# Gabriel-SGama/Semantic-SuperPoint

Hardware: AMD Instinct MI355X
Metric: image-pairs/sec at 240x320 bs32 (pair training step) (higher is better)
Workload: dtype f32

## Files before the change

include/ssp_hip.h:

```cpp
#ifndef SSP_HIP_H
#define SSP_HIP_H

#include <stddef.h>
#include <stdint.h>

#ifdef __cplusplus
extern "C" {
#endif

typedef struct ssp_handle ssp_handle;

enum { SSP_ARCH_GAUSS2 = 0, SSP_ARCH_GAUSS2_SSMALL = 1 };
enum { SSP_NREP = 32 };

typedef struct {
  int arch;
  int n_classes;
  int max_batch;
  int height;
  int width;
  int n_match;
  int n_non;
  int dense_loss;
} ssp_config;
// ... 231 lines not shown
                      int cap, int n_pairs, int pair_stride, float nn_thresh, void* workspace_dev, float* match_dev,
                      int32_t* n_match_dev, void* stream);

#define SSP_CLASS_NONE 255
int ssp_op_point_classes(const float* sout_nhwc_dev, int cs, int b, int h, int w, int n_classes, const float* pts_dev,
                         int pts_stride, const int32_t* count_dev, int cap, uint8_t* cls_dev, void* stream);
int ssp_point_classes(ssp_handle* h, int slot, int n, const float* pts_dev, int pts_stride, const int32_t* count_dev, int cap,
                      uint8_t* cls_dev, void* stream);
size_t ssp_filter_workspace_bytes(int n, int cap);
int ssp_op_filter_points(const float* pts_dev, const int32_t* count_dev, const float* desc_dev, const uint8_t* cls_dev,
                         const uint32_t keep_mask[8], int n, int cap, float* pts_out_dev, int32_t* count_out_dev,
                         float* desc_out_dev, uint8_t* cls_out_dev, void* workspace_dev, void* stream);
int ssp_match_two_way_classes(const float* desc1_dev, const int32_t* count1_dev, const float* desc2_dev,
                              const int32_t* count2_dev, const uint8_t* cls1_dev, const uint8_t* cls2_dev, int cap, int n_pairs,
                              int pair_stride, float nn_thresh, void* workspace_dev, float* match_dev, int32_t* n_match_dev,
                              void* stream);

int ssp_eval_repeatability(const double* pts1_dev, const int32_t* n1_dev, const double* pts2_dev, const int32_t* n2_dev,
                           int cap, int n_pairs, int pair_stride, const double* hom_dev, const double* hom_inv_dev,
                           int height, int width, int keep_k, double dist_thresh, double* out_dev, void* stream);
size_t ssp_eval_ransac_workspace_bytes(int cap, int n_pairs);
int ssp_eval_ransac(const double* pts1_dev, const double* pts2_dev, int cap, int n_pairs, int pair_stride,
                    const float* match_dev, const int32_t* n_match_dev, const uint64_t* seeds_dev, void* workspace_dev,
                    double* h_dev, uint8_t* mask_dev, int32_t* n_inlier_dev, int32_t* status_dev, double* ap_dev,
                    void* stream);

#define SSP_DET_EVAL_MAX_R2 64
#define SSP_DET_EVAL_STATE_WORDS 80
#define SSP_DET_EVAL_CURVE_TILE 1024
typedef struct ssp_det_eval_params {
  int32_t height, width;
  float remove_zero;
  int32_t r2;
  float prob_thresh;
  int32_t simplified;
} ssp_det_eval_params;
size_t ssp_det_eval_workspace_bytes(const ssp_det_eval_params* p, int b, int cap);
int ssp_op_det_tp_fp(const float* prob_dev, const void* labels_dev, int labels_u8, const ssp_det_eval_params* p, int b,
                     void* workspace_dev, int64_t* keys_dev, int64_t capacity, int64_t* state_dev, void* stream);
int ssp_op_det_tp_fp_points(const float* pts_dev, const int32_t* count_dev, int cap, const void* labels_dev, int labels_u8,
                            const ssp_det_eval_params* p, int b, void* workspace_dev, int64_t* keys_dev, int64_t capacity,
                            int64_t* state_dev, void* stream);
size_t ssp_det_pr_curve_workspace_bytes(int64_t n_records);
int ssp_op_det_pr_curve(const int64_t* sorted_keys_dev, int64_t n_records, const int64_t* state_dev, void* workspace_dev,
                        float* prob_dev, uint8_t* tp_dev, double* precision_dev, double* recall_dev, double* map_dev,
                        void* stream);

#define SSP_TRACK_MAX_LENGTH 16
size_t ssp_track_workspace_bytes(int max_length, int point_cap, int row_cap);
int ssp_op_track_update(const int32_t* ids_in_dev, const int32_t* tid_in_dev, const double* score_in_dev,
                        const int32_t* state_in_dev, const float* match_dev, const double* match_score64_dev,
                        const int32_t* n_match_dev, const int32_t* n_points_dev, int max_length, int point_cap, int row_cap,
                        void* workspace_dev, int32_t* ids_out_dev, int32_t* tid_out_dev, double* score_out_dev,
                        int32_t* state_out_dev, void* stream);
int ssp_op_track_select(const int32_t* ids_dev, const int32_t* tid_dev, const double* score_dev, const int32_t* state_dev,
                        int max_length, int row_cap, int min_length, void* workspace_dev, double* tracks_dev,
                        int32_t* n_tracks_dev, void* stream);
int ssp_op_track_points(const double* tracks_dev, const int32_t* n_tracks_dev, const double* pts_dev, const int32_t* state_dev,
                        int max_length, int point_cap, int track_cap, int first_slot, double* xy_dev, void* stream);

int ssp_op_bn_bwd(const float* y_dev, const float* dout_dev, const float* gamma_dev, const float* stats4_dev,
                  float* dy_dev, float* dgamma_dev, float* dbeta_dev, float* dbias_dev, double* sums_dev, int n, int h,
                  int w, int c, int relu, int pool, void* stream);
int ssp_op_bn_bwd_strided(const float* y_dev, const float* dout_dev, const float* gamma_dev, const float* stats4_dev,
                          float* dy_dev, float* dgamma_dev, float* dbeta_dev, float* dbias_dev, double* sums_dev, int n,
                          int h, int w, int c, int cs, int relu, int pool, void* stream);

int ssp_set_conv_algo(int algo);
int ssp_handle_set_conv_algo(ssp_handle* h, int algo);

int ssp_debug_conv_knobs(int ablate, int grid);
int ssp_debug_occupancy(int which);

int ssp_debug_buffer(ssp_handle* h, int slot, const char* name, float** ptr, size_t* nfloats);

int ssp_debug_backward_taps(ssp_handle* h, float* arena_dev, size_t arena_floats, unsigned layer_mask);
size_t ssp_debug_backward_tap_floats(const ssp_handle* h, unsigned layer_mask);
int ssp_debug_backward_tap(ssp_handle* h, int slot, int layer, int which, size_t* offset, size_t* nfloats, unsigned* route);

int ssp_op_sparse_loss(const float* desc_a_nhwc_dev, const float* desc_b_nhwc_dev, const int32_t* match_a_dev,
                       const int32_t* match_b_dev, const int32_t* nonmatch_b_dev, int b, int hc, int wc, int n_match,
                       int n_non, int method, int dist, float coef_pos, float coef_neg, float* dd_a_nhwc_dev, float* dd_b_nhwc_dev,
                       float* out2_dev, void* stream);

int ssp_op_dense_loss(const float* desc_a_nhwc_dev, const float* desc_b_nhwc_dev, const float* homographies_dev,
                      const float* valid_dev, int b, int hc, int wc, float lamda_d, float descriptor_dist, int multi_task,
                      float scale, void* scratch_dev, size_t scratch_bytes, float* out3_dev, float* dda_dev,
                      float* ddb_dev, void* stream);

#ifdef __cplusplus
}
#endif
#endif
```

semantic-superpoint_amd/csrc/bn_kernels.hip.h:

```cpp
#pragma once
#include <hip/hip_runtime.h>
#include <stdint.h>

#include "conv_mfma.hip.h"

namespace sspk {

template <typename T>
__device__ __forceinline__ float4 ld4(const T* p) {
  if constexpr (sizeof(T) == 4) {
    return *reinterpret_cast<const float4*>(p);
  } else {
    const u32x2 v = *reinterpret_cast<const u32x2*>(p);
    return make_float4(bf16_lo(v[0]), bf16_hi(v[0]), bf16_lo(v[1]), bf16_hi(v[1]));
  }
}
template <typename T>
__device__ __forceinline__ void st4(T* p, float4 v) {
  if constexpr (sizeof(T) == 4) {
    *reinterpret_cast<float4*>(p) = v;
  } else {
    u32x2 o;
    o[0] = pack_bf16(v.x, v.y);
    o[1] = pack_bf16(v.z, v.w);
// ... 684 lines not shown
      for (int o = 16; o > 0; o >>= 1) part += __shfl_xor(part, o);
      s2 = part;
    }
    if (!writer) continue;
    const float k1 = (float)(s1 / a.count), k2 = (float)(s2 / a.count);
    float* k12 = const_cast<float*>(a.k12);
    k12[c] = k1;
    k12[C + c] = k2;
    if (dbeta != nullptr) dbeta[c] += (float)s1;
    if (dgamma != nullptr) dgamma[c] += (float)s2;
    if (a.dbias != nullptr) a.dbias[c] += a.gamma[c] * a.invstd[c] * (float)(s1 - a.count * (double)k1);
  }
}
template <typename T = float>
__global__ void bn_bwd_sums_kernel(const BnBwdArgs a0, const BnBwdArgs a1, int nviews, float* __restrict__ dgamma,
                                   float* __restrict__ dbeta) {
  bn_bwd_sums_body<T>(a0, a1, nviews, dgamma, dbeta);
}
struct BnSumsJobs {
  BnBwdArgs a0[3], a1[3];
  float* dgamma[3];
  float* dbeta[3];
  int n;
};
template <typename T = float>
__global__ void bn_bwd_sums_multi_kernel(const BnSumsJobs J, int nviews) {
  const int j = blockIdx.y;
  bn_bwd_sums_body<T>(J.a0[j], J.a1[j], nviews, J.dgamma[j], J.dbeta[j]);
}

__global__ void nhwc_affine_to_nchw_kernel(const float* __restrict__ y, const float* __restrict__ scale,
                                           const float* __restrict__ shift, float* __restrict__ out, int N, int HW,
                                           int C, int cs, int co) {
  const long idx = (long)blockIdx.x * blockDim.x + threadIdx.x;
  if (idx >= (long)N * C * HW) return;
  const int p = (int)(idx % HW);
  const int c = (int)((idx / HW) % C);
  const int n = (int)(idx / ((long)HW * C));
  float v = y[((size_t)n * HW + p) * cs + co + c];
  if (scale != nullptr) v = fmaf(v, scale[c], shift[c]);
  out[idx] = v;
}

__global__ void nchw_to_nhwc_kernel(const float* __restrict__ in, float* __restrict__ out, int N, int HW, int C, int cs,
                                    int co) {
  const long idx = (long)blockIdx.x * blockDim.x + threadIdx.x;
  if (idx >= (long)N * C * HW) return;
  const int c = (int)(idx % C);
  const int p = (int)((idx / C) % HW);
  const int n = (int)(idx / ((long)HW * C));
  out[((size_t)n * HW + p) * cs + co + c] = in[((size_t)n * C + c) * HW + p];
}

__global__ __launch_bounds__(256) void desc_normalize_kernel(const float* __restrict__ y0, const float* __restrict__ scale0,
                                                             const float* __restrict__ shift0, float* __restrict__ desc0,
                                                             float* __restrict__ inv_norm0, float* __restrict__ zero_out0, int ncells,
                                                             int cs, int co, const float* __restrict__ y1 = nullptr,
                                                             const float* __restrict__ scale1 = nullptr,
                                                             const float* __restrict__ shift1 = nullptr, float* __restrict__ desc1 = nullptr,
                                                             float* __restrict__ inv_norm1 = nullptr, float* __restrict__ zero_out1 = nullptr) {
  const bool v1 = blockIdx.y != 0;
  const float* __restrict__ y = v1 ? y1 : y0;
  const float* __restrict__ scale = v1 ? scale1 : scale0;
  const float* __restrict__ shift = v1 ? shift1 : shift0;
  float* __restrict__ desc = v1 ? desc1 : desc0;
  float* __restrict__ inv_norm = v1 ? inv_norm1 : inv_norm0;
  float* __restrict__ zero_out = v1 ? zero_out1 : zero_out0;
  const int wave = (blockIdx.x * blockDim.x + threadIdx.x) >> 6;
  const int lane = threadIdx.x & 63;
  if (wave >= ncells) return;
  if (zero_out != nullptr) *reinterpret_cast<float4*>(zero_out + (size_t)wave * 256 + lane * 4) = make_float4(0.f, 0.f, 0.f, 0.f);
  const float4 v = *reinterpret_cast<const float4*>(y + (size_t)wave * cs + co + lane * 4);
  const float4 sc = *reinterpret_cast<const float4*>(scale + lane * 4);
  const float4 sh = *reinterpret_cast<const float4*>(shift + lane * 4);
  float4 r = make_float4(fmaf(v.x, sc.x, sh.x), fmaf(v.y, sc.y, sh.y), fmaf(v.z, sc.z, sh.z), fmaf(v.w, sc.w, sh.w));
  float s = r.x * r.x + r.y * r.y + r.z * r.z + r.w * r.w;
#pragma unroll
  for (int o = 32; o > 0; o >>= 1) s += __shfl_xor(s, o);
  const float inv = 1.f / sqrtf(s);
  *reinterpret_cast<float4*>(desc + (size_t)wave * 256 + lane * 4) = make_float4(r.x * inv, r.y * inv, r.z * inv, r.w * inv);
  if (lane == 0) inv_norm[wave] = inv;
}

__global__ __launch_bounds__(256) void desc_normalize_bwd_kernel(const float* __restrict__ desc0,
                                                                 const float* __restrict__ inv_norm0,
                                                                 float* __restrict__ d0, int ncells,
                                                                 const float* __restrict__ desc1 = nullptr,
                                                                 const float* __restrict__ inv_norm1 = nullptr,
                                                                 float* __restrict__ d1 = nullptr) {
  const bool v1 = blockIdx.y != 0;
  const float* __restrict__ desc = v1 ? desc1 : desc0;
  const float* __restrict__ inv_norm = v1 ? inv_norm1 : inv_norm0;
  float* __restrict__ d = v1 ? d1 : d0;
  const int wave = (blockIdx.x * blockDim.x + threadIdx.x) >> 6;
  const int lane = threadIdx.x & 63;
  if (wave >= ncells) return;
  const float4 n = *reinterpret_cast<const float4*>(desc + (size_t)wave * 256 + lane * 4);
  float4 g = *reinterpret_cast<const float4*>(d + (size_t)wave * 256 + lane * 4);
  float s = n.x * g.x + n.y * g.y + n.z * g.z + n.w * g.w;
#pragma unroll
  for (int o = 32; o > 0; o >>= 1) s += __shfl_xor(s, o);
  const float inv = inv_norm[wave];
  g = make_float4((g.x - n.x * s) * inv, (g.y - n.y * s) * inv, (g.z - n.z * s) * inv, (g.w - n.w * s) * inv);
  *reinterpret_cast<float4*>(d + (size_t)wave * 256 + lane * 4) = g;
}

__global__ void adam_kernel(float* __restrict__ p, const float* __restrict__ g, float* __restrict__ m,
                            float* __restrict__ v, long n, float step_size, float bc2_sqrt) {
  const long i = (long)blockIdx.x * blockDim.x + threadIdx.x;
  if (i >= n) return;
  const float gi = g[i];
  const float mi = 0.9f * m[i] + 0.1f * gi;
  const float vi = 0.999f * v[i] + 0.001f * gi * gi;
  m[i] = mi;
  v[i] = vi;
  const float denom = sqrtf(vi) / bc2_sqrt + 1e-8f;
  p[i] -= step_size * (mi / denom);
}

__global__ void adam_scaled_kernel(float* __restrict__ p, const float* __restrict__ g, float* __restrict__ m,
                                   float* __restrict__ v, long n, float step_size, float bc2_sqrt, float gscale) {
  const long i = (long)blockIdx.x * blockDim.x + threadIdx.x;
  if (i >= n) return;
  const float gi = g[i] * gscale;
  const float mi = 0.9f * m[i] + 0.1f * gi;
  const float vi = 0.999f * v[i] + 0.001f * gi * gi;
  m[i] = mi;
  v[i] = vi;
  const float denom = sqrtf(vi) / bc2_sqrt + 1e-8f;
  p[i] -= step_size * (mi / denom);
}

}
```

semantic-superpoint_amd/csrc/loss_kernels.hip.h:

```cpp
#pragma once
#include <hip/hip_runtime.h>
#include <stdint.h>

#include "det.hip.h"

namespace sspk {

template <typename Op>
__device__ __forceinline__ float wave_reduce(float v, float identity, Op op) {
  auto dpp = [&](float x, int ctrl_sel) {
    const int xi = __float_as_int(x), idn = __float_as_int(identity);
    int r;
    switch (ctrl_sel) {
      case 0: r = __builtin_amdgcn_update_dpp(idn, xi, 0xB1, 0xF, 0xF, false); break;
      case 1: r = __builtin_amdgcn_update_dpp(idn, xi, 0x4E, 0xF, 0xF, false); break;
      case 2: r = __builtin_amdgcn_update_dpp(idn, xi, 0x141, 0xF, 0xF, false); break;
      case 3: r = __builtin_amdgcn_update_dpp(idn, xi, 0x140, 0xF, 0xF, false); break;
      case 4: r = __builtin_amdgcn_update_dpp(idn, xi, 0x142, 0xA, 0xF, false); break;
      default: r = __builtin_amdgcn_update_dpp(idn, xi, 0x143, 0xC, 0xF, false); break;
    }
    return __int_as_float(r);
  };
  v = op(v, dpp(v, 0));
  v = op(v, dpp(v, 1));
// ... 114 lines not shown
    const int cx = cell % Wc, cy = (cell / Wc) % Hc, n = cell / (Wc * Hc);
    const float lab = labels2d[((size_t)n * H + cy * 8 + (lane >> 3)) * W + cx * 8 + (lane & 7)];
    const float lsum = wave_sum(lab);
    float dust = 1.f - lsum;
    if (dust < 1.f) dust = 0.f;
    const float dn = lsum + dust;
    const float t = lab / dn, td = dust / dn;
    const float* yp = ypb + (size_t)cell * cs;
    const float s = fmaf(yp[lane], sc_l, sh_l);
    const float sd = fmaf(yp[64], sc_d, sh_d);
    const float mx = fmaxf(wave_max(s), sd);
    const float e = expf(s - mx), ed = expf(sd - mx);
    const float inv = 1.f / (wave_sum(e) + ed);
    const float p = e * inv, pd = ed * inv;
    const float l = -(t * fmaxf(logf(p), -100.f) + (1.f - t) * fmaxf(log1pf(-p), -100.f));
    const float ld = -(td * fmaxf(logf(pd), -100.f) + (1.f - td) * fmaxf(log1pf(-pd), -100.f));
    const float m = cellmask[cell];
    lsum_acc += (wave_sum(l) + ld) * m;
    if (dsemi != nullptr) {
      const float coef = coef0 * m;
      const float g = (p - t) / fmaxf(p * (1.f - p), 1e-12f);
      const float gd = (pd - td) / fmaxf(pd * (1.f - pd), 1e-12f);
      const float dot = wave_sum(g * p) + gd * pd;
      float* dp = dsemi + (size_t)cell * cs;
      dp[lane] = coef * p * (g - dot);
      if (lane == 0) dp[64] = coef * pd * (gd - dot);
      if (lane >= 1 && lane < cs - 64) dp[64 + lane] = 0.f;
    }
  }
  const float tot = block_sum_of_waves(lsum_acc, red);
  if (threadIdx.x == 0) acc_add_loss(&acc->det_sum[view], (double)tot);
}

struct Bilin {
  int i00, i01, i10, i11;
  float w00, w01, w10, w11;
};
__device__ __forceinline__ Bilin bilin_setup(int cell, int Hc, int Wc) {
  const float u = (float)(cell % Wc), v = (float)(cell / Wc);
  const float gx = u / (float)Wc * 2.f - 1.f, gy = v / (float)Hc * 2.f - 1.f;
  const float ix = ((gx + 1.f) / 2.f) * (float)(Wc - 1), iy = ((gy + 1.f) / 2.f) * (float)(Hc - 1);
  const float fx = floorf(ix), fy = floorf(iy);
  const int x0 = (int)fx, y0 = (int)fy, x1 = x0 + 1, y1 = y0 + 1;
  const float ax = ix - fx, ay = iy - fy;
  Bilin b;
  const bool vx0 = x0 >= 0 && x0 < Wc, vx1 = x1 >= 0 && x1 < Wc, vy0 = y0 >= 0 && y0 < Hc, vy1 = y1 >= 0 && y1 < Hc;
  const int cx0 = min(max(x0, 0), Wc - 1), cx1 = min(max(x1, 0), Wc - 1);
  const int cy0 = min(max(y0, 0), Hc - 1), cy1 = min(max(y1, 0), Hc - 1);
  b.i00 = cy0 * Wc + cx0; b.i01 = cy0 * Wc + cx1; b.i10 = cy1 * Wc + cx0; b.i11 = cy1 * Wc + cx1;
  b.w00 = (vx0 && vy0) ? (1.f - ax) * (1.f - ay) : 0.f;
  b.w01 = (vx1 && vy0) ? ax * (1.f - ay) : 0.f;
  b.w10 = (vx0 && vy1) ? (1.f - ax) * ay : 0.f;
  b.w11 = (vx1 && vy1) ? ax * ay : 0.f;
  return b;
}
__device__ __forceinline__ Bilin bilin_cell(int cell) {
  Bilin b;
  b.i00 = b.i01 = b.i10 = b.i11 = cell;
  b.w00 = 1.f; b.w01 = b.w10 = b.w11 = 0.f;
  return b;
}
constexpr int DESC_METHOD_1D = 1;
constexpr int DESC_EUCLIDEAN = 2;
__device__ __forceinline__ float4 f4_fma(float w, float4 a, float4 acc) {
  return make_float4(fmaf(w, a.x, acc.x), fmaf(w, a.y, acc.y), fmaf(w, a.z, acc.z), fmaf(w, a.w, acc.w));
}
__device__ __forceinline__ void atomic_add4(float* p, float4 v) {
  facc_add(p, v.x);
  facc_add(p + 1, v.y);
  facc_add(p + 2, v.z);
  facc_add(p + 3, v.w);
}


static inline int desc_grid(int B, int n_match) { return ((B + 7) / 8) * 8 * ((n_match + 3) / 4); }
__device__ __forceinline__ int desc_wave_of_block(int B, int n_match, int& img) {
  const int bpi = (n_match + 3) >> 2;
  const int xcd = blockIdx.x & 7, slot = blockIdx.x >> 3;
  const int round = slot / bpi;
  img = round * 8 + xcd;
  const int k = (slot - round * bpi) * 4 + (threadIdx.x >> 6);
  return (img < B && k < n_match) ? img * n_match + k : -1;
}
template <bool BWD, bool EUC = false>
__global__ __launch_bounds__(256) void desc_match_kernel(const float* __restrict__ desc_a, const float* __restrict__ desc_b,
                                                         const int32_t* __restrict__ match_a,
                                                         const int32_t* __restrict__ match_b, float* __restrict__ dd_a,
                                                         float* __restrict__ dd_b, StepAccum* __restrict__ acc, int B,
                                                         int Hc, int Wc, int n_match, int flags) {
  const DetTarget t_a = det_resolve(dd_a), t_b = det_resolve(dd_b);
  int img;
  const int w = desc_wave_of_block(B, n_match, img);
  const int lane = threadIdx.x & 63;
  if (w < 0) return;
  const bool m1d = (flags & DESC_METHOD_1D) != 0;
  constexpr bool euc = EUC;
  const size_t base = (size_t)img * Hc * Wc * 256 + lane;
  const Bilin ba = m1d ? bilin_cell(match_a[w]) : bilin_setup(match_a[w], Hc, Wc);
  const Bilin bb = m1d ? bilin_cell(match_b[w]) : bilin_setup(match_b[w], Hc, Wc);
  float va[4] = {0.f, 0.f, 0.f, 0.f}, vb[4] = {0.f, 0.f, 0.f, 0.f};
  const int ia[4] = {ba.i00, ba.i01, ba.i10, ba.i11}, ib[4] = {bb.i00, bb.i01, bb.i10, bb.i11};
  const float wa[4] = {ba.w00, ba.w01, ba.w10, ba.w11}, wb[4] = {bb.w00, bb.w01, bb.w10, bb.w11};
  if (m1d) {
#pragma unroll
    for (int j = 0; j < 4; ++j) {
      va[j] = desc_a[base + (size_t)ia[0] * 256 + 64 * j];
      vb[j] = desc_b[base + (size_t)ib[0] * 256 + 64 * j];
    }
  } else {
#pragma unroll
    for (int k = 0; k < 4; ++k)
#pragma unroll
      for (int j = 0; j < 4; ++j) {
        va[j] = fmaf(wa[k], desc_a[base + (size_t)ia[k] * 256 + 64 * j], va[j]);
        vb[j] = fmaf(wb[k], desc_b[base + (size_t)ib[k] * 256 + 64 * j], vb[j]);
      }
  }
  float term;
  if (!euc) {
    term = fmaxf(1.f - wave_sum(va[0] * vb[0] + va[1] * vb[1] + va[2] * vb[2] + va[3] * vb[3]), 0.f);
  } else {
    float q = 0.f;
#pragma unroll
    for (int j = 0; j < 4; ++j) q = fmaf(va[j] - vb[j], va[j] - vb[j], q);
    term = wave_sum(q);
  }
  if (lane == 0) acc_add_loss(&acc->pos_sum[img * 16 + ((w >> 2) & 15)], (double)term);
  if (BWD && (euc || term > 0.f)) {
    const float c = acc->coef_pos / ((float)n_match * (float)B) * (euc ? 2.f : -1.f);
#pragma unroll
    for (int k = 0; k < 4; ++k) {
      if (wa[k] != 0.f) {
#pragma unroll
        for (int j = 0; j < 4; ++j) facc_add(t_a, dd_a + base + (size_t)ia[k] * 256 + 64 * j, wa[k] * c * (euc ? va[j] - vb[j] : vb[j]));
      }
      if (wb[k] != 0.f) {
#pragma unroll
        for (int j = 0; j < 4; ++j) facc_add(t_b, dd_b + base + (size_t)ib[k] * 256 + 64 * j, wb[k] * c * (euc ? vb[j] - va[j] : va[j]));
      }
    }
  }
}

template <bool EUC = false>
__global__ __launch_bounds__(256) void desc_nonmatch_fwd_kernel(const float* __restrict__ desc_a,
                                                                const float* __restrict__ desc_b,
                                                                const int32_t* __restrict__ match_a,
                                                                const int32_t* __restrict__ nonmatch_b,
                                                                float* __restrict__ dots, StepAccum* __restrict__ acc,
                                                                int B, int Hc, int Wc, int n_match, int n_non, int flags) {
  int img;
  const int w = desc_wave_of_block(B, n_match, img);
  const int lane = threadIdx.x & 63;
  if (w < 0) return;
  constexpr bool euc = EUC;
  (void)flags;
  const int grp = lane >> 4, l16 = lane & 15;
  const size_t ibase = (size_t)img * Hc * Wc * 256;
  const float* ap = desc_a + ibase + (size_t)match_a[w] * 256 + l16 * 4;
  float4 a[4];
#pragma unroll
  for (int i = 0; i < 4; ++i) a[i] = *reinterpret_cast<const float4*>(ap + i * 64);
  float hsum = 0.f;
  unsigned cnt = 0;
  const int32_t* nm = nonmatch_b + (size_t)w * n_non;
  for (int j0 = 0; j0 < n_non; j0 += 4) {
    const int j = j0 + grp;
    const bool valid = j < n_non;
    const int bi = valid ? nm[j] : 0;
    const float* bp = desc_b + ibase + (size_t)bi * 256 + l16 * 4;
    float d = 0.f;
#pragma unroll
    for (int i = 0; i < 4; ++i) {
      const float4 b = *reinterpret_cast<const float4*>(bp + i * 64);
      if (!euc) {
        d += a[i].x * b.x + a[i].y * b.y + a[i].z * b.z + a[i].w * b.w;
      } else {
        const float ex = a[i].x - b.x, ey = a[i].y - b.y, ez = a[i].z - b.z, ew = a[i].w - b.w;
        d += ex * ex + ey * ey + ez * ez + ew * ew;
      }
    }
#pragma unroll
    for (int o = 8; o > 0; o >>= 1) d += __shfl_xor(d, o);
    if (euc) d = sqrtf(d);
    if (l16 == 0 && valid) {
      if (dots != nullptr) dots[(size_t)w * n_non + j] = d;
      float h = fmaxf(d - 0.2f, 0.f);
      if (euc) h *= h;
      hsum += h;
      cnt += (h != 0.f) ? 1u : 0u;
    }
  }
  hsum = wave_sum(hsum);
  const float c = wave_sum((float)cnt);
  if (lane == 0) {
    const int rep = img * 16 + ((w >> 2) & 15);
    acc_add_loss(&acc->neg_sum[rep], (double)hsum);
    atomicAdd(&acc->nnz[rep], (unsigned)(c + 0.5f));
  }
}

template <bool EUC = false>
__global__ __launch_bounds__(256) void desc_nonmatch_bwd_kernel(const float* __restrict__ desc_a,
                                                                const float* __restrict__ desc_b,
                                                                const int32_t* __restrict__ match_a,
                                                                const int32_t* __restrict__ nonmatch_b,
                                                                const float* __restrict__ dots, float* __restrict__ dd_a,
                                                                float* __restrict__ dd_b, const StepAccum* __restrict__ acc,
                                                                int B, int Hc, int Wc, int n_match, int n_non, int flags) {
  constexpr bool euc = EUC;
  (void)flags;
  const DetTarget t_a = det_resolve(dd_a), t_b = det_resolve(dd_b);
  int img;
  const int w = desc_wave_of_block(B, n_match, img);
  const int lane = threadIdx.x & 63;
  if (w < 0) return;
  const size_t ibase = (size_t)img * Hc * Wc * 256 + lane;
  const float wgt = acc->coef_neg / (((float)nnz_of_image(acc, img) + 1.f) * (float)B);
  const int32_t* nm = nonmatch_b + (size_t)w * n_non;
  const float* dk = dots + (size_t)w * n_non;
  const int ma = match_a[w];
  float a[4], ga[4] = {0.f, 0.f, 0.f, 0.f};
  bool have_a = false;
// ... 185 lines not shown
```

semantic-superpoint_amd/csrc/ssp.hip:

```cpp
#include "../../include/ssp_hip.h"

#include <hip/hip_runtime.h>

#include <cmath>
#include <cstdarg>
#include <cstdio>
#include <cstdlib>
#include <algorithm>
#include <cstring>
#include <string>
#include <vector>

#include "bn_kernels.hip.h"
#include "conv_mfma.hip.h"
#include "conv1x1_group.hip.h"
#include "conv_wino.hip.h"
#include "conv_wino_pipe.hip.h"
#include "conv_wino_p2.hip.h"
#include "conv_wino4.hip.h"
#include "wgrad_wino4.hip.h"
#include "wgrad_wino_fused.hip.h"
#include "conv_bf16.hip.h"
#include "conv_bf16_ws.hip.h"
#include "wgrad_bf16.hip.h"
// ... 62 lines not shown
    if (done[dev]) return false;
    done[dev] = true;
    return true;
  }
};

static inline int cdiv(long a, long b) { return (int)((a + b - 1) / b); }
static int device_cu_count() {
  static int cached[64] = {};
  int dev = 0;
  if (hipGetDevice(&dev) != hipSuccess || dev < 0 || dev >= 64) return 256;
  if (cached[dev] == 0) {
    int n = 0;
    cached[dev] = (hipDeviceGetAttribute(&n, hipDeviceAttributeMultiprocessorCount, dev) == hipSuccess && n > 0) ? n : 256;
  }
  return cached[dev];
}
static inline size_t align_up(size_t v, size_t a) { return (v + a - 1) / a * a; }

struct LayerDesc {
  int cin, cout, ks;
  bool bn;
  size_t w_off, b_off, g_off, be_off;
  int bn_index;
  size_t bn_ch_off;
  size_t pk_fwd, pk_bwd;
  int nchunks_fwd, ncob_fwd, nchunks_bwd, ncob_bwd;
};

struct BnBufs {
  double* stats;
  double* bsums;
  float *scale, *shift, *mean, *invstd;
  float* k12;
};

struct Slot {
  float* Y[16];
  int y_cs[16], y_co[16];
  BnBufs bn[16];
  float* desc;
  float* inv_norm;
  float* cellmask;
  float* dsemi;
  float* ddesc;
  float* dsout;
  float *gP, *gQ;
  float* Apool[8];
  bool pool_raw[8] = {false, false, false, false, false, false, false, false};
  float* act[8] = {nullptr, nullptr, nullptr, nullptr, nullptr, nullptr, nullptr, nullptr};
  bool act_valid[8] = {false, false, false, false, false, false, false, false};
  const float* x;
  void* stats_region;
  size_t stats_bytes;
  int N, H, W;
  bool bsums_dirty;
  bool has_desc;
};

struct ssp_handle {
  ssp_config cfg;
  int nlayers, nheads;
  LayerDesc L[16];
  size_t n_params, n_bn_ch;
  int n_bn;
  ssp_buffers buf;
  bool bound;
  size_t ws_bytes;
  Slot slot[2];
  float *wpk_fwd, *wpk_bwd, *wpk_heads_bwd;
  float* partial;
  size_t partial_floats;
  size_t partial_used = 0;
  struct WredBQueue* rq_bf16 = nullptr;
  WredJobs rjobs{};
  bool bsums_fused[16] = {};
  bool sums_lazy[16] = {};
  bool fin_pending[16] = {};
  double fin_count[16] = {};
  bool apply_fused[16] = {};
  bool bf16_fuse_apply = true;
  StepAccum* accum;
  float* dots;
  float* dense_coef;
  int sout_cs;
  int conv_algo;
  bool pk_w4_fwd[16] = {}, pk_w4_bwd[16] = {};
  float *wpk_g1_fwd[16] = {}, *wpk_g1_bwd[16] = {};
  bool pk_g1[16] = {};
  float* g1_partial = nullptr;
  TailJobs tail = {};
  int g1_partial_slabs = 0;
  int packed_algo = -1;
  bool packed_bwd = false;
  struct GraphEntry { std::vector<unsigned char> key; hipGraphExec_t exec; };
  std::vector<GraphEntry> graphs;
  uint64_t* graph_seed;
  hipStream_t aux_stream = nullptr;
  hipStream_t aux2_stream = nullptr;
  hipEvent_t ev_fork = nullptr, ev_join = nullptr;
  hipEvent_t ev_pack_fork = nullptr, ev_pack_join = nullptr;
  hipEvent_t ev_early_fork = nullptr, ev_early_join = nullptr;
  int prof_family;
  bool prof_paused = false;
  std::vector<hipEvent_t> ev_pool;
  size_t ev_used;
  double prof_flops, prof_bytes, prof_exec_flops;
  int64_t prof_launches;
  struct ProfKernel { double flops = 0, exec_flops = 0, bytes = 0; int64_t launches = 0; } prof_k[SSP_PROF_K_COUNT];
  std::vector<unsigned char> ev_kernel;
  int n_cu;
  float* tap_arena = nullptr;
  unsigned tap_mask = 0;
  unsigned tap_route[16] = {};
  int tap_wk = 0, tap_dk = 0;
};

enum { TAP_BSUMS_FUSED = 1, TAP_APPLY_FUSED = 2, TAP_SUMS_LAZY = 4, TAP_ACT_INPUT = 8, TAP_WG_SHIFT = 4, TAP_DG_SHIFT = 8 };
enum { TAP_WG_FUSED12 = 1, TAP_WG_WINO = 2, TAP_WG_WINO4 = 3, TAP_WG_DIRECT = 4, TAP_WG_GROUPED = 5, TAP_WG_L0 = 6, TAP_WG_BF16 = 7 };
enum { TAP_DG_WINO4 = 1, TAP_DG_PIPE = 2, TAP_DG_P2 = 3, TAP_DG_DIRECT = 4, TAP_DG_GROUPED = 5, TAP_DG_BF16 = 6, TAP_DG_BF16_WS = 7 };

struct AlgoScope {
  int prev;
  explicit AlgoScope(const ssp_handle* h) : prev(g_conv_algo) { g_conv_algo = h ? h->conv_algo : g_default_conv_algo; }
  ~AlgoScope() { g_conv_algo = prev; }
};

enum { L_PA = 8, L_PB = 9, L_DA = 10, L_DB = 11, L_DS = 12, L_SOUT = 13 };
static const int kEnc[8][2] = {{1, 64}, {64, 64}, {64, 64}, {64, 64}, {64, 128}, {128, 128}, {128, 128}, {128, 128}};

static void build_layers(ssp_handle* h) {
  int n = 0;
  auto add = [&](int cin, int cout, int ks, bool bn) {
    LayerDesc& d = h->L[n++];
    d.cin = cin; d.cout = cout; d.ks = ks; d.bn = bn;
  };
  for (int i = 0; i < 8; ++i) add(kEnc[i][0], kEnc[i][1], 3, true);
  add(128, 256, 3, true);
  add(256, 65, 1, true);
  add(128, 256, 3, true);
  add(256, 256, 1, true);
  h->nheads = 2;
  if (h->cfg.arch == SSP_ARCH_GAUSS2_SSMALL) {
    add(128, 256, 3, true);
    add(256, h->cfg.n_classes, 1, false);
    h->nheads = 3;
  }
  h->nlayers = n;
  size_t off = 0, bnch = 0, pf = 0, pb = 0;
  int nbn = 0;
  for (int i = 0; i < n; ++i) {
    LayerDesc& d = h->L[i];
    d.w_off = off; off += (size_t)d.cout * d.cin * d.ks * d.ks;
    d.b_off = off; off += d.cout;
    if (d.bn) {
      d.g_off = off; off += d.cout;
      d.be_off = off; off += d.cout;
      d.bn_index = nbn++;
      d.bn_ch_off = bnch; bnch += d.cout;
    } else {
      d.g_off = d.be_off = 0; d.bn_index = -1; d.bn_ch_off = 0;
    }
    const int taps = d.ks * d.ks;
    d.nchunks_fwd = cdiv(d.cin, CK); d.ncob_fwd = cdiv(d.cout, NB);
    d.nchunks_bwd = cdiv(d.cout, CK); d.ncob_bwd = cdiv(d.cin, NB);
    (void)taps;
// ... 28 lines not shown
    T* p = base ? reinterpret_cast<T*>(base + off) : nullptr;
    off += n * sizeof(T);
    return p;
  }
};

static size_t carve(ssp_handle* h, void* base) {
  Carver c{reinterpret_cast<char*>(base), 0};
  const int B = h->cfg.max_batch, H = h->cfg.height, W = h->cfg.width;
  const size_t cells = (size_t)B * (H / 8) * (W / 8);
  h->sout_cs = (int)align_up(h->cfg.n_classes, 4);
  size_t pf = 0, pb = 0;
  for (int i = 0; i < h->nlayers; ++i) {
    const LayerDesc& d = h->L[i];
    pf = d.pk_fwd + (size_t)d.ncob_fwd * d.nchunks_fwd * pk_taps(d.ks) * CK * NB;
    pb = d.pk_bwd + (size_t)d.ncob_bwd * d.nchunks_bwd * pk_taps(d.ks) * CK * NB;
  }
  h->wpk_fwd = c.take<float>(pf);
  h->wpk_bwd = c.take<float>(pb);
  h->wpk_heads_bwd = c.take<float>((size_t)2 * 16 * h->nheads * WC * CK * NB);
  for (int i = 0; i < h->nlayers; ++i) {
    const LayerDesc& d = h->L[i];
    h->wpk_g1_fwd[i] = h->wpk_g1_bwd[i] = nullptr;
    if (d.ks != 1) continue;
    h->wpk_g1_fwd[i] = c.take<float>((size_t)cdiv(d.cin, G1_KC) * cdiv(d.cout, 32) * G1_TILE_FLOATS);
    h->wpk_g1_bwd[i] = c.take<float>((size_t)cdiv(d.cout, G1_KC) * cdiv(d.cin, 32) * G1_TILE_FLOATS);
  }
  h->g1_partial_slabs = 2 * std::max(h->n_cu, 8);
  h->g1_partial = c.take<float>((size_t)h->g1_partial_slabs * G1W_SLAB);
  for (int s = 0; s < 2; ++s) {
    Slot& S = h->slot[s];
    for (int l = 0; l < 8; ++l) {
      int lh, lw; layer_res(l, H, W, lh, lw);
      S.Y[l] = c.take_skewed<float>((size_t)B * lh * lw * h->L[l].cout);
      S.y_cs[l] = h->L[l].cout; S.y_co[l] = 0;
    }
    for (int l = 0; l < 8; ++l) S.Apool[l] = nullptr;
    for (int l = 1; l <= 5; l += 2) {
      int lh, lw; layer_res(l, H, W, lh, lw);
      S.Apool[l] = c.take_skewed<float>((size_t)B * (lh / 2) * (lw / 2) * h->L[l].cout);
    }
    const int hcs = 256 * h->nheads;
    float* yheads = c.take_skewed<float>(cells * hcs);
    S.Y[L_PA] = yheads; S.y_cs[L_PA] = hcs; S.y_co[L_PA] = 0;
    S.Y[L_DA] = yheads; S.y_cs[L_DA] = hcs; S.y_co[L_DA] = 256;
    S.Y[L_PB] = c.take_skewed<float>(cells * 80); S.y_cs[L_PB] = 80; S.y_co[L_PB] = 0;
    S.Y[L_DB] = c.take_skewed<float>(cells * 256); S.y_cs[L_DB] = 256; S.y_co[L_DB] = 0;
    if (h->nheads == 3) {
      S.Y[L_DS] = yheads; S.y_cs[L_DS] = hcs; S.y_co[L_DS] = 512;
      S.Y[L_SOUT] = c.take<float>(cells * h->sout_cs); S.y_cs[L_SOUT] = h->sout_cs; S.y_co[L_SOUT] = 0;
      S.dsout = c.take<float>(cells * h->sout_cs);
    } else {
      S.dsout = nullptr;
    }
    S.desc = c.take_skewed<float>(cells * 256);
    for (int l = 5; l <= 7; ++l) S.act[l] = c.take_skewed<float>(cells * 64);
    S.inv_norm = c.take<float>(cells);
    S.cellmask = c.take<float>(cells);
    S.dsemi = c.take<float>(cells * 80);
    S.ddesc = c.take_skewed<float>(cells * 256);
    size_t nst = 0;
    for (int l = 0; l < h->nlayers; ++l) nst += 4 * (size_t)h->L[l].cout * NREP;
    double* st = c.take<double>(nst);
    S.stats_region = st; S.stats_bytes = nst * sizeof(double);
    for (int l = 0; l < h->nlayers; ++l) {
      const int C = h->L[l].cout;
      S.bn[l].stats = st; st += 2 * C * NREP;
      S.bn[l].bsums = st; st += 2 * C * NREP;
      S.bn[l].scale = c.take<float>(C); S.bn[l].shift = c.take<float>(C);
      S.bn[l].mean = c.take<float>(C); S.bn[l].invstd = c.take<float>(C);
      S.bn[l].k12 = c.take<float>(2 * C);
    }
  }
  const size_t big = (size_t)B * H * W * 64;
  for (int s = 0; s < 2; ++s) {
    h->slot[s].gP = c.take_skewed<float>(big);
    h->slot[s].gQ = c.take_skewed<float>(big);
  }
  h->partial_floats = (size_t)1024 * 9 * 4096 * 5;
  h->partial = c.take<float>(h->partial_floats);
  h->accum = c.take<StepAccum>(1);
  h->graph_seed = c.take<uint64_t>(1);
  h->dots = c.take<float>((size_t)B * h->cfg.n_match * h->cfg.n_non);
  {
    const size_t pc = (size_t)(H / 8) * (W / 8);
    h->dense_coef = h->cfg.dense_loss ? c.take_skewed<float>((size_t)std::min(B, 64) * pc * pc) : nullptr;
  }
  return align_up(c.off, 256) + (base ? 0 : ((size_t)4 << 20));
}

struct ProfScope {
  ssp_handle* h; hipStream_t st; bool on;
  ProfScope(ssp_handle* h_, int family, hipStream_t s, double flops, double bytes, double exec_flops = -1.0,
            int kernel = SSP_PROF_K_OTHER) : h(h_), st(s), on(false) {
    const bool conv = family == SSP_PROF_CONV3X3_FWD || family == SSP_PROF_CONV3X3_DGRAD;
    const bool match = h && family > 0 && !h->prof_paused && (h->prof_family == family || (h->prof_family == SSP_PROF_CONV3X3_ALL && conv) ||
        (h->prof_family == SSP_PROF_CONV3X3_EVERY && (conv || family == SSP_PROF_CONV3X3_WGRAD)));
    if (match && h->ev_used + 2 <= h->ev_pool.size()) {
      on = true;
      (void)hipEventRecord(h->ev_pool[h->ev_used], st);
      const double ex = exec_flops >= 0.0 ? exec_flops : flops;
      h->prof_flops += flops; h->prof_bytes += bytes; h->prof_launches += 1;
      h->prof_exec_flops += ex;
      ssp_handle::ProfKernel& k = h->prof_k[kernel];
      k.flops += flops; k.exec_flops += ex; k.bytes += bytes; k.launches += 1;
      h->ev_kernel[h->ev_used / 2] = (unsigned char)kernel;
    }
  }
  ~ProfScope() {
    if (on) { (void)hipEventRecord(h->ev_pool[h->ev_used + 1], st); h->ev_used += 2; }
  }
};

__global__ void zero_fill_kernel(uint32_t* __restrict__ p0, size_t nwords, uint32_t* __restrict__ p1 = nullptr) {
  uint32_t* __restrict__ p = blockIdx.y ? p1 : p0;
  const size_t tid = (size_t)blockIdx.x * blockDim.x + threadIdx.x, nth = (size_t)gridDim.x * blockDim.x;
  if ((reinterpret_cast<size_t>(p) & 15) == 0) {
    uint4* q = reinterpret_cast<uint4*>(p);
    const size_t nq = nwords >> 2;
    for (size_t i = tid; i < nq; i += nth) q[i] = make_uint4(0u, 0u, 0u, 0u);
    for (size_t i = (nq << 2) + tid; i < nwords; i += nth) p[i] = 0u;
  } else {
    for (size_t i = tid; i < nwords; i += nth) p[i] = 0u;
  }
}
static int dev_zero(void* p, size_t bytes, hipStream_t st) {
  if (bytes == 0) return 0;
  if (bytes % 4 != 0 || (reinterpret_cast<size_t>(p) & 3) != 0) return fail(-1, "dev_zero: unaligned range");
  const size_t nwords = bytes / 4;
  const int nb = (int)std::min<size_t>((nwords / 4 + 255) / 256 + 1, 2048);
  hipLaunchKernelGGL(zero_fill_kernel, dim3(nb), dim3(256), 0, st, reinterpret_cast<uint32_t*>(p), nwords);
  HIPCHK(hipGetLastError());
  return 0;
}
static int dev_zero2(void* p0, void* p1, size_t bytes, hipStream_t st) {
  if (bytes == 0) return 0;
  if (p1 == nullptr || p1 == p0) return dev_zero(p0, bytes, st);
  if (bytes % 4 != 0 || ((reinterpret_cast<size_t>(p0) | reinterpret_cast<size_t>(p1)) & 3) != 0) return fail(-1, "dev_zero2: unaligned range");
  const size_t nwords = bytes / 4;
  const int nb = (int)std::min<size_t>((nwords / 4 + 255) / 256 + 1, 2048);
  hipLaunchKernelGGL(zero_fill_kernel, dim3(nb, 2), dim3(256), 0, st, reinterpret_cast<uint32_t*>(p0), nwords, reinterpret_cast<uint32_t*>(p1));
  HIPCHK(hipGetLastError());
  return 0;
}

template <int KS, int IN_MODE, int SH, int SW>
static int launch_conv_t(const ConvArgs& a, int nblocks, hipStream_t st) {
  using G = ConvGeom<KS, SH, SW>;
  static AttrOnce attr_once;
  auto kern = conv_mfma_kernel<KS, IN_MODE, SH, SW>;
  if (attr_once.need()) {
    HIPCHK(hipFuncSetAttribute(reinterpret_cast<const void*>(kern), hipFuncAttributeMaxDynamicSharedMemorySize, G::LDS_BYTES));
  }
  hipLaunchKernelGGL(kern, dim3(nblocks), dim3(256), G::LDS_BYTES, st, a);
  HIPCHK(hipGetLastError());
  return 0;
}

struct ConvCall {
  const float* in; int in_cs, in_co, cin;
  const float* wpk; const float* bias;
  float* out; int out_cs, out_co, cout;
  const float* in_scale; const float* in_shift; double* stats;
  int N, H, W, ks, in_mode, nchunks, ncob;
  int nprob = 1;
  const float* in2 = nullptr; float* out2 = nullptr;
// ... 593 lines not shown
  const int taps = ks * ks;
  const int conv_cin = tf ? cout_w : cin_w, conv_cout = tf ? cin_w : cout_w;
  const int nchunks = cdiv(conv_cin, CK), ncob = cdiv(conv_cout, NB);
  if (wino) {
    const int total = ncob * nchunks * WB_FLOATS;
    if (w4)
      hipLaunchKernelGGL(pack_weights_wino4_kernel, dim3(cdiv(ncob * 2 * nchunks * W4_B_FLOATS, 256)), dim3(256), 0, st, w, dst,
                         cout_w, cin_w, tf, 2 * nchunks, 0, 0, ncob, 2 * nchunks);
    else
      hipLaunchKernelGGL(pack_weights_wino8_kernel, dim3(cdiv(total, 256)), dim3(256), 0, st, w, dst, cout_w, cin_w, tf,
                         2 * nchunks, 0, 0, ncob, 2 * nchunks);
    HIPCHK(hipGetLastError());
    return 0;
  }
  const int total = ncob * nchunks * taps * CK * NB;
  hipLaunchKernelGGL(pack_weights_kernel, dim3(cdiv(total, 256)), dim3(256), 0, st, w, dst, cout_w, cin_w, ks, tf,
                     nchunks, 0, 0, ncob, nchunks);
  HIPCHK(hipGetLastError());
  return 0;
}

struct BnPlainJob {
  BnBwdArgs a[2];
  float* dg = nullptr;
  float* db = nullptr;
  bool filled = false;
};
struct BnSumsQueue {
  BnSumsJobs J;
  int maxC = 0;
  BnSumsQueue() { J.n = 0; }
};
static int flush_bn_sums(BnSumsQueue& q, int nviews, hipStream_t st) {
  if (q.J.n == 0) return 0;
  if (q.J.n == 1) hipLaunchKernelGGL(bn_bwd_sums_kernel<float>, dim3(cdiv(q.maxC * 32, 256)), dim3(256), 0, st, q.J.a0[0], q.J.a1[0], nviews,
                                     q.J.dgamma[0], q.J.dbeta[0]);
  else hipLaunchKernelGGL(bn_bwd_sums_multi_kernel<float>, dim3(cdiv(q.maxC * 32, 256), q.J.n), dim3(256), 0, st, q.J, nviews);
  HIPCHK(hipGetLastError());
  q.J.n = 0; q.maxC = 0;
  return 0;
}
template <bool RELU, bool POOL, typename T = float>
static int launch_bn_bwd(const BnBwdArgs* a, int nviews, float* dgamma, float* dbeta, hipStream_t st,
                         bool sums_done = false, bool skip_apply = false, BnSumsQueue* queue = nullptr) {
  if (queue != nullptr && sums_done && skip_apply && (sizeof(T) == 4 || a[0].pool_fix == 0) && queue->J.n < 3) {
    const int j = queue->J.n++;
    queue->J.a0[j] = a[0]; queue->J.a1[j] = a[nviews - 1]; queue->J.dgamma[j] = dgamma; queue->J.dbeta[j] = dbeta;
    queue->maxC = std::max(queue->maxC, a[0].C);
    return 0;
  }
  const BnBwdArgs& a0 = a[0];
  const BnBwdArgs& a1 = a[nviews - 1];
  const int nq = (a0.C + 3) / 4, rows = 256 / nq;
  const long npix = (long)a0.N * (POOL ? a0.H / 2 : a0.H) * (POOL ? a0.W / 2 : a0.W);
  int nb = cdiv(npix, rows);
  if (nb > 1024) nb = 1024;
  if (!sums_done)
    hipLaunchKernelGGL((bn_bwd_kernel<RELU, POOL, false, T>), dim3(nb, nviews), dim3(256), 0, st, a0, a1, a0, a1);
  hipLaunchKernelGGL(bn_bwd_sums_kernel<T>, dim3(cdiv(a0.C * 32, 256)), dim3(256), 0, st, a0, a1, nviews, dgamma, dbeta);
  if (!skip_apply)
    hipLaunchKernelGGL((bn_bwd_kernel<RELU, POOL, true, T>), dim3(nb, nviews), dim3(256), 0, st, a0, a1, a0, a1);
  HIPCHK(hipGetLastError());
  return 0;
}

template <typename K>
static int l0_resident_grid(K kern, const ssp_handle* h, int nviews, long rows, int W) {
  static int per_cu = 0, per_cu_w = 0;
  if (per_cu_w != W) { per_cu = 0; per_cu_w = W; }
  if (per_cu == 0 && (hipOccupancyMaxActiveBlocksPerMultiprocessor(&per_cu, kern, 256, l0_lds_bytes(W)) != hipSuccess || per_cu < 1)) {
    (void)hipGetLastError();
    per_cu = -1;
  }
  if (per_cu < 1) return l0_grid(rows);
  const long g = std::max(1L, (long)per_cu * (h ? h->n_cu : 256) / std::max(1, nviews));
  return (int)std::min(rows, g);
}

#include "bf16_host.hip.h"

static int flush_wgrad_reduce_bf16(ssp_handle* h, hipStream_t st) { return h->rq_bf16 != nullptr ? h->rq_bf16->flush(st) : 0; }

static int ensure_aux_stream(ssp_handle* h);

struct DetHostRegion { float* lo; size_t n; long long* shadow; const ssp_handle* owner; };
static std::vector<DetHostRegion> g_det_regions;
static int g_det_mode = -1;
static int g_det_device = -1;
static bool det_mode() {
  if (g_det_mode < 0) { const char* e = getenv("SSP_DETERMINISTIC"); g_det_mode = (e != nullptr && atoi(e) != 0) ? 1 : 0; }
  return g_det_mode == 1;
}
static int det_upload() {
  DetRegion tab[DET_MAX_REGIONS];
  int n = 0;
  for (const DetHostRegion& r : g_det_regions) {
    if (n == DET_MAX_REGIONS) return fail(-3, "deterministic mode: more than %d fp32 scatter targets are bound in this process", DET_MAX_REGIONS);
    tab[n].lo = r.lo; tab[n].hi = r.lo + r.n; tab[n].shadow = r.shadow; ++n;
  }
  for (int i = n; i < DET_MAX_REGIONS; ++i) { tab[i].lo = tab[i].hi = nullptr; tab[i].shadow = nullptr; }
  const int flag = det_mode() ? 1 : 0;
  HIPCHK(hipMemcpyToSymbol(HIP_SYMBOL(g_det_region), tab, sizeof(tab)));
  HIPCHK(hipMemcpyToSymbol(HIP_SYMBOL(g_det_nregion), &n, sizeof(n)));
  HIPCHK(hipMemcpyToSymbol(HIP_SYMBOL(g_det), &flag, sizeof(flag)));
  return 0;
}
static void det_release(const ssp_handle* h) {
  bool any = false;
  for (size_t i = 0; i < g_det_regions.size();) {
    if (g_det_regions[i].owner == h) { (void)hipFree(g_det_regions[i].shadow); g_det_regions.erase(g_det_regions.begin() + i); any = true; }
    else ++i;
  }
  if (any && det_upload() != 0) fprintf(stderr, "libssp_hip: deterministic-mode region table upload failed on release: %s\n", g_err.c_str());
}
static int det_register(const ssp_handle* h, float* lo, size_t n) {
  if (lo == nullptr || n == 0) return 0;
  DetHostRegion r;
  r.lo = lo; r.n = n; r.owner = h; r.shadow = nullptr;
  HIPCHK(hipMalloc(&r.shadow, n * sizeof(long long)));
  HIPCHK(hipMemset(r.shadow, 0, n * sizeof(long long)));
  g_det_regions.push_back(r);
  return 0;
}
static int det_fold(float* base, hipStream_t st) {
  if (!det_mode() || base == nullptr) return 0;
  for (const DetHostRegion& r : g_det_regions)
    if (r.lo == base) {
      hipLaunchKernelGGL(det_fold_kernel, dim3((unsigned)std::min<long>(cdiv((long)r.n, 256), 2048)), dim3(256), 0, st, r.shadow, r.lo, (long)r.n);
      HIPCHK(hipGetLastError());
      return 0;
    }
  return 0;
}

extern "C" {

const char* ssp_last_error(void) { return g_err.c_str(); }

#ifndef SSP_BUILD_ID
#define SSP_BUILD_ID "unknown"
#endif
const char* ssp_build_id(void) {
  static const char marker[] = "SSP_BUILD_ID=" SSP_BUILD_ID;
  return marker + 13;
}

__global__ __launch_bounds__(256) void clock_probe_kernel(float* sink, unsigned long long* out, int iters) {
  f32x16 acc[4];
#pragma unroll
  for (int i = 0; i < 4; ++i)
#pragma unroll
    for (int r = 0; r < 16; ++r) acc[i][r] = 0.f;
  float a[4], b[4];
  unsigned s = threadIdx.x * 2654435761u + blockIdx.x * 40503u + 12345u;
#pragma unroll
  for (int i = 0; i < 4; ++i) {
    s = s * 1664525u + 1013904223u; a[i] = ((int)(s >> 8) - (1 << 23)) * (1.f / (1 << 23));
    s = s * 1664525u + 1013904223u; b[i] = ((int)(s >> 8) - (1 << 23)) * (0.05f / (1 << 23));
  }
  const unsigned long long c0 = __builtin_readcyclecounter(), r0 = __builtin_amdgcn_s_memrealtime();
  for (int it = 0; it < iters; ++it) {
#pragma unroll
    for (int u = 0; u < 4; ++u)
#pragma unroll
      for (int m = 0; m < 4; ++m) acc[m] = __builtin_amdgcn_mfma_f32_32x32x2f32(a[m], b[(m + u) & 3], acc[m], 0, 0, 0);
  }
  const unsigned long long c1 = __builtin_readcyclecounter(), r1 = __builtin_amdgcn_s_memrealtime();
  float r = 0.f;
#pragma unroll
  for (int i = 0; i < 4; ++i) r += acc[i][0] + acc[i][9];
  sink[blockIdx.x * 256 + threadIdx.x] = r;
  if (blockIdx.x == 0 && threadIdx.x == 0) { out[0] = c1 - c0; out[1] = r1 - r0; }
}

int ssp_clock_probe(float ms, double* mhz_out, void* stream_) {
  hipStream_t stream = (hipStream_t)stream_;
  if (!mhz_out || !(ms > 0.f) || ms > 1000.f) return fail(-1, "ssp_clock_probe: bad argument");
  int dev = 0, ncu = 256;
  if (hipGetDevice(&dev) != hipSuccess || hipDeviceGetAttribute(&ncu, hipDeviceAttributeMultiprocessorCount, dev) != hipSuccess)
    return fail(-2, "ssp_clock_probe: no device");
  float* sink = nullptr;
  unsigned long long* out = nullptr;
  if (hipMalloc(&sink, (size_t)ncu * 256 * 4) != hipSuccess) return fail(-2, "ssp_clock_probe: hipMalloc");
  if (hipMalloc(&out, 16) != hipSuccess) { (void)hipFree(sink); return fail(-2, "ssp_clock_probe: hipMalloc"); }
  const int iters = (int)(ms * 2.4e6f / 1024.f) + 1;
  unsigned long long h[2] = {0, 0};
  hipLaunchKernelGGL(clock_probe_kernel, dim3(ncu), dim3(256), 0, stream, sink, out, iters);
  hipError_t e = hipMemcpyAsync(h, out, 16, hipMemcpyDeviceToHost, stream);
  if (e == hipSuccess) e = hipStreamSynchronize(stream);
  (void)hipFree(sink);
  (void)hipFree(out);
  if (e != hipSuccess || h[1] == 0) return fail(-2, "ssp_clock_probe: %s", hipGetErrorString(e));
  *mhz_out = 100.0 * (double)h[0] / (double)h[1];
  return 0;
}

__global__ void idle_kernel(unsigned long long ticks) {
  const unsigned long long t0 = __builtin_amdgcn_s_memrealtime();
  while (__builtin_amdgcn_s_memrealtime() - t0 < ticks) __builtin_amdgcn_s_sleep(127);
}

int ssp_set_deterministic(int on) {
  g_det_mode = on ? 1 : 0;
  return det_upload();
}
int ssp_get_deterministic(void) { return det_mode() ? 1 : 0; }

int ssp_create(const ssp_config* cfg, ssp_handle** out) {
  if (!cfg || !out) return fail(-1, "null argument");
  if (cfg->arch != SSP_ARCH_GAUSS2 && cfg->arch != SSP_ARCH_GAUSS2_SSMALL) return fail(-1, "unknown arch %d", cfg->arch);
  if (cfg->height % 8 || cfg->width % 8 || cfg->height <= 0 || cfg->width <= 0)
    return fail(-1, "height/width must be positive multiples of 8 (got %dx%d)", cfg->height, cfg->width);
  if (cfg->width > L0_MAX_W) return fail(-1, "width must be <= %d (row images of the first-layer kernels)", L0_MAX_W);
  if (cfg->max_batch < 1 || cfg->max_batch > 1024) return fail(-1, "max_batch must be in 1..1024");
  if (cfg->arch == SSP_ARCH_GAUSS2_SSMALL && cfg->n_classes > 192) return fail(-1, "n_classes must be <= 192");
  ssp_handle* h = new ssp_handle();
  h->cfg = *cfg;
  if (h->cfg.n_classes <= 0) h->cfg.n_classes = 133;
  if (h->cfg.n_match <= 0) h->cfg.n_match = 1000;
  if (h->cfg.n_non <= 0) h->cfg.n_non = 100;
  h->conv_algo = g_default_conv_algo;
  h->rq_bf16 = new WredBQueue();
  AlgoScope algo(h);
  build_layers(h);
  h->bound = false;
  h->n_cu = device_cu_count();
  h->ws_bytes = carve(h, nullptr);
  h->prof_family = 0; h->ev_used = 0; h->prof_flops = h->prof_bytes = h->prof_exec_flops = 0; h->prof_launches = 0;
  *out = h;
  return 0;
}

void ssp_destroy(ssp_handle* h) {
  if (!h) return;
  det_release(h);
  delete h->rq_bf16;
  for (auto e : h->ev_pool) (void)hipEventDestroy(e);
  for (auto& g : h->graphs) (void)hipGraphExecDestroy(g.exec);
  if (h->ev_fork) (void)hipEventDestroy(h->ev_fork);
  if (h->ev_join) (void)hipEventDestroy(h->ev_join);
  if (h->ev_pack_fork) (void)hipEventDestroy(h->ev_pack_fork);
  if (h->ev_pack_join) (void)hipEventDestroy(h->ev_pack_join);
  if (h->ev_early_fork) (void)hipEventDestroy(h->ev_early_fork);
  if (h->ev_early_join) (void)hipEventDestroy(h->ev_early_join);
  if (h->aux_stream) (void)hipStreamDestroy(h->aux_stream);
  if (h->aux2_stream) (void)hipStreamDestroy(h->aux2_stream);
  delete h;
}

size_t ssp_param_count(const ssp_handle* h) { return h ? h->n_params : 0; }
size_t ssp_bn_channel_count(const ssp_handle* h) { return h ? h->n_bn_ch : 0; }
int ssp_bn_layer_count(const ssp_handle* h) { return h ? h->n_bn : 0; }
size_t ssp_workspace_bytes(const ssp_handle* h) { return h ? h->ws_bytes : 0; }

int ssp_bind(ssp_handle* h, const ssp_buffers* b, void* stream) {
  if (!h || !b) return fail(-1, "null argument");
  if (!b->params_dev || !b->bn_running_dev || !b->workspace_dev) return fail(-1, "params, bn_running and workspace are required");
  if (b->workspace_bytes < h->ws_bytes) return fail(-1, "workspace too small: %zu < %zu", b->workspace_bytes, h->ws_bytes);
  h->buf = *b;
  for (auto& g : h->graphs) (void)hipGraphExecDestroy(g.exec);
  h->graphs.clear();
  carve(h, b->workspace_dev);
  CHK(ensure_aux_stream(h));
  HIPCHK(hipMemsetAsync(b->workspace_dev, 0, h->ws_bytes, (hipStream_t)stream));
  det_release(h);
  if (det_mode()) {
    int dev_now = -1;
    HIPCHK(hipGetDevice(&dev_now));
    if (g_det_device >= 0 && g_det_device != dev_now && !g_det_regions.empty())
      return fail(-3, "deterministic mode: handles of ONE device per process (regions of device %d are bound, this bind is on device %d)", g_det_device, dev_now);
    const int need = (b->grads_dev ? 1 : 0) + 2 + (h->slot[0].dsout ? 2 : 0);
    if ((int)g_det_regions.size() + need > DET_MAX_REGIONS)
      return fail(-3, "deterministic mode: %d fp32 scatter targets are bound in this process, this handle needs %d more (limit %d)",
                  (int)g_det_regions.size(), need, DET_MAX_REGIONS);
    g_det_device = dev_now;
    const size_t cells = (size_t)h->cfg.max_batch * (h->cfg.height / 8) * (h->cfg.width / 8);
    int rc = det_register(h, b->grads_dev, b->grads_dev ? h->n_params + 3 : 0);
    for (int v = 0; v < 2 && rc == 0; ++v) {
      rc = det_register(h, h->slot[v].ddesc, cells * 256);
      if (rc == 0) rc = det_register(h, h->slot[v].dsout, h->slot[v].dsout ? cells * h->sout_cs : 0);
    }
    if (rc == 0) rc = det_upload();
    if (rc != 0) { det_release(h); return rc; }
  }
  h->bound = true;
  return 0;
}

int ssp_zero_grad(ssp_handle* h, void* stream) {
  if (!h || !h->bound || !h->buf.grads_dev) return fail(-1, "handle not bound with a gradient buffer");
  CHK(dev_zero(h->buf.grads_dev, (h->n_params + 3) * sizeof(float), (hipStream_t)stream));
  return 0;
}

int ssp_profile_enable(ssp_handle* h, int family) {
  if (!h) return fail(-1, "null handle");
  h->prof_family = family; h->ev_used = 0; h->prof_flops = h->prof_bytes = h->prof_exec_flops = 0; h->prof_launches = 0;
  h->prof_paused = false;
  for (auto& k : h->prof_k) k = ssp_handle::ProfKernel();
  if (family != 0 && h->ev_pool.empty()) {
    h->ev_pool.resize(8192);
    h->ev_kernel.assign(4096, (unsigned char)SSP_PROF_K_OTHER);
    for (auto& e : h->ev_pool) HIPCHK(hipEventCreate(&e));
  }
// ... 1130 lines not shown
  AlgoScope algo(h);
  if (n < 1 || n > h->cfg.max_batch || height > h->cfg.height || width > h->cfg.width || height % 8 || width % 8)
    return fail(-1, "forward shape [%d,1,%d,%d] exceeds the configured maximum or is not a multiple of 8", n, height, width);
  if ((size_t)height * width != (size_t)h->cfg.height * h->cfg.width && (size_t)n * height * width > (size_t)h->cfg.max_batch * h->cfg.height * h->cfg.width)
    return fail(-1, "forward shape too large");
  hipStream_t st = (hipStream_t)stream;
  {
    SlotSet SS{1, {&h->slot[slot], nullptr}};
    const float* xs[2] = {x_dev, nullptr};
    CHK(run_forward(h, SS, xs, n, height, width, train, h->buf.grads_dev != nullptr, st));
  }
  Slot& S = h->slot[slot];
  const int HW = (height / 8) * (width / 8);
  if (semi_dev) {
    const long tot = (long)n * 65 * HW;
    hipLaunchKernelGGL(nhwc_affine_to_nchw_kernel, dim3(cdiv(tot, 256)), dim3(256), 0, st, S.Y[L_PB], S.bn[L_PB].scale,
                       S.bn[L_PB].shift, semi_dev, n, HW, 65, 80, 0);
  }
  if (desc_dev) {
    const long tot = (long)n * 256 * HW;
    hipLaunchKernelGGL(nhwc_affine_to_nchw_kernel, dim3(cdiv(tot, 256)), dim3(256), 0, st, S.desc, (const float*)nullptr,
                       (const float*)nullptr, desc_dev, n, HW, 256, 256, 0);
  }
  if (sem_dev) {
    if (h->nheads != 3) return fail(-1, "sem output requested from a model without a segmentation head");
    const long tot = (long)n * h->cfg.n_classes * height * width;
    hipLaunchKernelGGL(sem_upsample_nchw_kernel, dim3(cdiv(tot, 256)), dim3(256), 0, st, S.Y[L_SOUT], sem_dev, n,
                       height / 8, width / 8, height, width, h->cfg.n_classes, h->sout_cs);
  }
  HIPCHK(hipGetLastError());
  return 0;
}

int ssp_backward(ssp_handle* h, int slot, const float* dsemi_dev, const float* ddesc_dev, const float* dsem_dev,
                 void* stream) {
  if (!h || !h->bound || !h->buf.grads_dev) return fail(-1, "handle not bound with a gradient buffer");
  if (slot < 0 || slot > 1) return fail(-1, "slot must be 0 or 1");
  AlgoScope algo(h);
  hipStream_t st = (hipStream_t)stream;
  Slot& S = h->slot[slot];
  const int N = S.N, Hc = S.H / 8, Wc = S.W / 8, HW = Hc * Wc, ncells = N * HW;
  const float *ds = nullptr, *dd = nullptr, *dso = nullptr;
  if (dsemi_dev) {
    const long tot = (long)N * 65 * HW;
    hipLaunchKernelGGL(nchw_to_nhwc_kernel, dim3(cdiv(tot, 256)), dim3(256), 0, st, dsemi_dev, S.dsemi, N, HW, 65, 80, 0);
    ds = S.dsemi;
  }
  if (ddesc_dev) {
    const long tot = (long)N * 256 * HW;
    hipLaunchKernelGGL(nchw_to_nhwc_kernel, dim3(cdiv(tot, 256)), dim3(256), 0, st, ddesc_dev, S.ddesc, N, HW, 256, 256, 0);
    hipLaunchKernelGGL(desc_normalize_bwd_kernel, dim3(cdiv(ncells, 4)), dim3(256), 0, st, S.desc, S.inv_norm, S.ddesc, ncells);
    dd = S.ddesc;
  }
  if (dsem_dev) {
    if (h->nheads != 3) return fail(-1, "dsem given for a model without a segmentation head");
    CHK(dev_zero(S.dsout, (size_t)ncells * h->sout_cs * sizeof(float), st));
    const long tot = (long)N * h->cfg.n_classes * Hc * Wc;
    hipLaunchKernelGGL(sem_upsample_bwd_nchw_kernel, dim3(cdiv(tot, 256)), dim3(256), 0, st, dsem_dev, S.dsout, N, Hc, Wc,
                       S.H, S.W, h->cfg.n_classes, h->sout_cs);
    dso = S.dsout;
  }
  HIPCHK(hipGetLastError());
  SlotSet SS{1, {&h->slot[slot], nullptr}};
  const float* dss[2] = {ds, nullptr};
  const float* dds[2] = {dd, nullptr};
  float* dsos[2] = {const_cast<float*>(dso), nullptr};
  return run_backward(h, SS, dss, dds, dsos, st);
}

int ssp_adam_step(ssp_handle* h, float lr, int step, void* stream) {
  if (!h || !h->bound || !h->buf.grads_dev || !h->buf.adam_m_dev || !h->buf.adam_v_dev)
    return fail(-1, "handle not bound with gradient and Adam state buffers");
  if (step < 1) return fail(-1, "Adam step index starts at 1");
  const long n = (long)h->n_params + 3;
  const AdamScalars a = adam_scalars(lr, step);
  hipLaunchKernelGGL(adam_kernel, dim3(cdiv(n, 256)), dim3(256), 0, (hipStream_t)stream, h->buf.params_dev,
                     h->buf.grads_dev, h->buf.adam_m_dev, h->buf.adam_v_dev, n, a.step_size, a.bc2_sqrt);
  HIPCHK(hipGetLastError());
  return 0;
}

}

static int sem_xc_env() {
  static const int v = [] { const char* e = getenv("SSP_SEM_XC"); return e ? atoi(e) : 1; }();
  return v;
}
static int launch_sem_ce(int algo, bool train, const float* sout, const int64_t* labels, float* dsout, StepAccum* acc, int view, int B,
                         int Hc, int Wc, int H, int W, int C, int cs, hipStream_t st, const float* sout1 = nullptr,
                         const int64_t* labels1 = nullptr, float* dsout1 = nullptr) {
  const bool xc_ok = H == 8 * Hc && W == 8 * Wc && C <= 16 * SEMX_NB;
  if (algo == 2 && !xc_ok) return fail(-1, "sem_ce: the (x, class) form needs H = 8 Hc, W = 8 Wc and <= %d classes", 16 * SEMX_NB);
  if (C > SEM_MAX_C) return fail(-1, "sem_ce: at most %d classes", SEM_MAX_C);
  const bool xc = algo == 2 || (algo == 0 && xc_ok && sem_xc_env() != 0);
  const long ntile = (long)B * (Hc + 1) * (Wc + 1);
  const int nviews = sout1 != nullptr ? 2 : 1;
  if (xc) {
    static const int wgs_per_cu = [] { const char* e = getenv("SSP_SEM_XC_WGS"); return e ? atoi(e) : 2; }();
    const SemXcGeom geom = sem_xc_geom(B, Hc, Wc, wgs_per_cu * device_cu_count());
    const int grid = B * geom.row_groups * geom.x_splits * nviews;
#define SSP_SEM_XC(MODE, NB) \
  hipLaunchKernelGGL((sem_ce_xc_kernel<MODE, NB>), dim3(grid), dim3(256), 0, st, sout, labels, dsout, acc, view, B, Hc, Wc, C, cs, geom, sout1, \
                     labels1, dsout1)
    if (train) { if (C <= 48) SSP_SEM_XC(3, 3); else if (C <= 96) SSP_SEM_XC(3, 6); else SSP_SEM_XC(3, 9); }
    else { if (C <= 48) SSP_SEM_XC(1, 3); else if (C <= 96) SSP_SEM_XC(1, 6); else SSP_SEM_XC(1, 9); }
#undef SSP_SEM_XC
  } else {
    const int grid = (int)std::min<long>((ntile + 3) / 4, 4096);
    for (int v = 0; v < nviews; ++v) {
      const float* so = v ? sout1 : sout; const int64_t* la = v ? labels1 : labels; float* ds = v ? dsout1 : dsout;
      if (train) hipLaunchKernelGGL((sem_ce_kernel<3>), dim3(grid), dim3(256), 0, st, so, la, ds, acc, view + v, B, Hc, Wc, H, W, C, cs);
      else hipLaunchKernelGGL((sem_ce_kernel<1>), dim3(grid), dim3(256), 0, st, so, la, ds, acc, view + v, B, Hc, Wc, H, W, C, cs);
    }
  }
  return 0;
}

static int pair_step_impl(ssp_handle* h, const ssp_pair_inputs* in, float* scalars_dev, int phase, hipStream_t st_in) {
  void* stream = st_in;
  if (!h || !h->bound) return fail(-1, "handle not bound");
  if (!in || !scalars_dev) return fail(-1, "null argument");
  if (phase < 0 || phase > 2) return fail(-1, "pair-step phase must be 0, 1 or 2");
  AlgoScope algo(h);
  const int nv = in && in->warped_image_dev ? 2 : 1;
  if (phase == 2) {
    if (!in->train) return 0;
    SlotSet SS2{nv, {&h->slot[0], nv == 2 ? &h->slot[1] : nullptr}};
    const float* none[2] = {nullptr, nullptr};
    float* nonef[2] = {nullptr, nullptr};
    return run_backward(h, SS2, none, none, nonef, (hipStream_t)stream, 2);
  }
  if (in->train && !h->buf.grads_dev) return fail(-1, "train step needs a gradient buffer");
  const int B = in->batch, H = h->cfg.height, W = h->cfg.width, Hc = H / 8, Wc = W / 8;
  if (B < 1 || B > h->cfg.max_batch || B > SSP_MAX_PAIRS)
    return fail(-1, "pair-step batch %d out of range (1..min(max_batch, %d))", B, SSP_MAX_PAIRS);
  const bool semantic = h->nheads == 3;
  if (semantic && (!in->semantic_dev || (nv == 2 && !in->warped_semantic_dev))) return fail(-1, "semantic labels required for the ssmall model");
  const bool use_desc = in->lambda_loss > 0.f;
  if (use_desc && nv == 1) return fail(-1, "need a pair of images: lambda_loss > 0 with warped_image_dev == NULL");
  if (!in->image_dev || !in->labels_dev || !in->valid_mask_dev || (nv == 2 && (!in->warped_labels_dev || !in->warped_valid_mask_dev)))
    return fail(-1, "pair step: image / labels / valid mask pointers of every view are required");
  const bool dense = use_desc && in->dense_loss != 0;
  if (dense && !h->dense_coef) return fail(-1, "dense descriptor loss needs a handle created with ssp_config.dense_loss = 1");
  if (use_desc && !dense && (!in->match_a_dev || !in->match_b_dev || !in->nonmatch_b_dev))
    return fail(-1, "sparse-loss indices required (call ssp_sample_indices or pass the reference's indices)");
  hipStream_t st = (hipStream_t)stream;
  const float* eta = h->buf.params_dev + h->n_params;
  const int ncells = B * Hc * Wc;
  hipLaunchKernelGGL(step_begin_kernel, dim3(1), dim3(64), 0, st, h->accum, eta, in->multi_task, in->lambda_loss,
                     in->lamda_d, (int)semantic, B);
  SlotSet SS{nv, {&h->slot[0], nv == 2 ? &h->slot[1] : nullptr}};
  static const int early_env = getenv("SSP_EARLY_LABELS") ? atoi(getenv("SSP_EARLY_LABELS")) : 1;
  const bool early = early_env != 0;
  const float* masks[2] = {in->valid_mask_dev, in->warped_valid_mask_dev};
  const int64_t* sems[2] = {in->semantic_dev, in->warped_semantic_dev};
  const bool zero_dsout = semantic && in->train;
  auto label_kernels = [&](hipStream_t se) -> int {
    hipLaunchKernelGGL(cell_mask_kernel, dim3(std::min(cdiv(ncells, 4), 512), nv), dim3(256), 0, se, masks[0], h->slot[0].cellmask,
                       &h->accum->mask_cnt[0], B, H, W, masks[nv - 1], h->slot[nv - 1].cellmask, &h->accum->mask_cnt[nv - 1]);
    if (semantic)
      hipLaunchKernelGGL(sem_count_kernel, dim3(512, nv), dim3(256), 0, se, sems[0], sems[1], (long)B * H * W, h->cfg.n_classes, h->accum,
                         zero_dsout ? h->slot[0].dsout : (float*)nullptr, zero_dsout && nv == 2 ? h->slot[1].dsout : (float*)nullptr,
                         (long)ncells * h->sout_cs);
    HIPCHK(hipGetLastError());
    return 0;
  };
  if (early) {
    CHK(ensure_aux_stream(h));
    HIPCHK(hipEventRecord(h->ev_early_fork, st));
    HIPCHK(hipStreamWaitEvent(h->aux2_stream, h->ev_early_fork, 0));
    CHK(label_kernels(h->aux2_stream));
    HIPCHK(hipEventRecord(h->ev_early_join, h->aux2_stream));
  }
  {
    const float* xs[2] = {in->image_dev, in->warped_image_dev};
    CHK(run_forward(h, SS, xs, B, H, W, 1, in->train != 0, st, false, early && in->train && use_desc && !dense));
  }
  if (early) HIPCHK(hipStreamWaitEvent(st, h->ev_early_join, 0));
  else CHK(label_kernels(st));
  {
    static const int idle_us = getenv("SSP_DBG_IDLE_US") ? atoi(getenv("SSP_DBG_IDLE_US")) : 0;
    if (idle_us > 0) hipLaunchKernelGGL(idle_kernel, dim3(1), dim3(64), 0, st, (unsigned long long)idle_us * 100ull);
  }
  static const int loss_stream_env = getenv("SSP_LOSS_STREAM") ? atoi(getenv("SSP_LOSS_STREAM")) : 1;
  hipStream_t sd = st;
  const bool forked = loss_stream_env != 0 && use_desc && !dense;
  SideFork loss_fork;
  if (forked) {
    CHK(ensure_aux_stream(h));
    sd = h->aux_stream;
    CHK(loss_fork.fork(st, sd, h->ev_fork, h->ev_join));
  }
  if (dense) {
    Slot &A = h->slot[0], &Bs = h->slot[1];
    const int pc = Hc * Wc;
    DenseArgs da;
    da.da = A.desc; da.db = Bs.desc; da.hn = in->homographies_dev; da.valid = Bs.cellmask;
    da.coef = in->train ? h->dense_coef : nullptr; da.acc = h->accum; da.B = B; da.Hc = Hc; da.Wc = Wc;
    da.lamda_d = in->dense_lamda_d; da.dist = in->descriptor_dist; da.multi_task = in->multi_task;
    hipLaunchKernelGGL(dense_dots_kernel, dim3(cdiv(pc, 64), cdiv(pc, 64), B), dim3(256), 0, sd, da);
    if (in->train) {
      hipLaunchKernelGGL((dense_grad_kernel<false>), dim3(4, cdiv(pc, 64), B), dim3(256), 0, sd, h->dense_coef, Bs.desc,
                         A.ddesc, pc);
      hipLaunchKernelGGL((dense_grad_kernel<true>), dim3(4, cdiv(pc, 64), B), dim3(256), 0, sd, h->dense_coef, A.desc,
                         Bs.ddesc, pc);
      hipLaunchKernelGGL(desc_normalize_bwd_kernel, dim3(cdiv(ncells, 4), 2), dim3(256), 0, sd, A.desc, A.inv_norm, A.ddesc, ncells,
                         Bs.desc, Bs.inv_norm, Bs.ddesc);
    }
    HIPCHK(hipGetLastError());
  } else if (use_desc) {
    Slot &A = h->slot[0], &Bs = h->slot[1];
    const int dflags = (in->sparse_method != 0 ? DESC_METHOD_1D : 0) | (in->sparse_dist != 0 ? DESC_EUCLIDEAN : 0);
    const bool euc = (dflags & DESC_EUCLIDEAN) != 0;
    const dim3 dgrid(desc_grid(B, h->cfg.n_match));
#define SSP_DESC(KERNEL, ...)                                                                 \
    {                                                                                         \
      if (euc) hipLaunchKernelGGL((KERNEL<true>), dgrid, dim3(256), 0, sd, __VA_ARGS__);      \
      else hipLaunchKernelGGL((KERNEL<false>), dgrid, dim3(256), 0, sd, __VA_ARGS__);         \
    }
#define SSP_DESC_MATCH(BWD, ...)                                                                        \
    {                                                                                                   \
      if (euc) hipLaunchKernelGGL((desc_match_kernel<BWD, true>), dgrid, dim3(256), 0, sd, __VA_ARGS__); \
      else hipLaunchKernelGGL((desc_match_kernel<BWD, false>), dgrid, dim3(256), 0, sd, __VA_ARGS__);   \
    }
    if (!in->train)
      SSP_DESC_MATCH(false, A.desc, Bs.desc, in->match_a_dev, in->match_b_dev, (float*)nullptr, (float*)nullptr, h->accum, B, Hc, Wc,
                     h->cfg.n_match, dflags)
    SSP_DESC(desc_nonmatch_fwd_kernel, A.desc, Bs.desc, in->match_a_dev, in->nonmatch_b_dev, in->train ? h->dots : (float*)nullptr, h->accum,
             B, Hc, Wc, h->cfg.n_match, h->cfg.n_non, dflags)
    if (in->train) {
      if (!early) {
        CHK(dev_zero(A.ddesc, (size_t)ncells * 256 * sizeof(float), sd));
        CHK(dev_zero(Bs.ddesc, (size_t)ncells * 256 * sizeof(float), sd));
      }
      SSP_DESC_MATCH(true, A.desc, Bs.desc, in->match_a_dev, in->match_b_dev, A.ddesc, Bs.ddesc, h->accum, B, Hc, Wc, h->cfg.n_match, dflags)
      SSP_DESC(desc_nonmatch_bwd_kernel, A.desc, Bs.desc, in->match_a_dev, in->nonmatch_b_dev, h->dots, A.ddesc, Bs.ddesc, h->accum, B, Hc, Wc,
               h->cfg.n_match, h->cfg.n_non, dflags)
#undef SSP_DESC
#undef SSP_DESC_MATCH
      CHK(det_fold(A.ddesc, sd));
      CHK(det_fold(Bs.ddesc, sd));
      hipLaunchKernelGGL(desc_normalize_bwd_kernel, dim3(cdiv(ncells, 4), 2), dim3(256), 0, sd, A.desc, A.inv_norm, A.ddesc, ncells,
                         Bs.desc, Bs.inv_norm, Bs.ddesc);
    }
    HIPCHK(hipGetLastError());
  }
  const float* labels[2] = {in->labels_dev, in->warped_labels_dev};
  {
    Slot &S = h->slot[0], &T = h->slot[nv - 1];
    hipLaunchKernelGGL(detector_loss_kernel, dim3(std::min(cdiv(ncells, 4), 1024), nv), dim3(256), 0, st, S.Y[L_PB], S.bn[L_PB].scale,
                       S.bn[L_PB].shift, labels[0], S.cellmask, in->train ? S.dsemi : nullptr, h->accum, 0, B, H, W, 80,
                       T.Y[L_PB], T.bn[L_PB].scale, T.bn[L_PB].shift, labels[nv - 1], T.cellmask, in->train ? T.dsemi : nullptr);
  }
  HIPCHK(hipGetLastError());
  if (semantic) {
    Slot &S = h->slot[0], &T = h->slot[nv - 1];
    CHK(launch_sem_ce(0, in->train != 0, S.Y[L_SOUT], sems[0], in->train ? S.dsout : nullptr, h->accum, 0, B, Hc, Wc, H, W, h->cfg.n_classes,
                      h->sout_cs, st, nv == 2 ? T.Y[L_SOUT] : nullptr, nv == 2 ? sems[1] : nullptr, nv == 2 && in->train ? T.dsout : nullptr));
    if (in->train)
      for (int v = 0; v < nv; ++v) CHK(det_fold(h->slot[v].dsout, st));
    HIPCHK(hipGetLastError());
  }
  CHK(loss_fork.join());
  hipLaunchKernelGGL(step_end_kernel, dim3(1), dim3(64), 0, st, h->accum, eta,
                     in->train ? h->buf.grads_dev + h->n_params : (float*)nullptr, scalars_dev, B, h->cfg.n_match,
                     in->multi_task, in->lambda_loss, in->lamda_d, (int)semantic, in->train, (int)dense, Hc * Wc, nv);
  HIPCHK(hipGetLastError());
  if (in->train) {
    const float* dss[2] = {h->slot[0].dsemi, nv == 2 ? h->slot[1].dsemi : nullptr};
    const float* dds[2] = {use_desc ? h->slot[0].ddesc : nullptr, use_desc ? h->slot[1].ddesc : nullptr};
    float* dsos[2] = {semantic ? h->slot[0].dsout : nullptr, semantic && nv == 2 ? h->slot[1].dsout : nullptr};
    CHK(run_backward(h, SS, dss, dds, dsos, st, phase));
  }
  return 0;
}

static int sample_indices_impl(ssp_handle* h, const float* homographies_dev, const float* hcell_dev, int batch, uint64_t seed,
                               const uint64_t* seed_dev, int32_t* match_a_dev, int32_t* match_b_dev, int32_t* nonmatch_b_dev,
                               hipStream_t st) {
  if (!h) return fail(-1, "null handle");
  if (!homographies_dev && !hcell_dev) return fail(-1, "sample_indices: homographies required");
  if (batch < 1 || batch > SSP_MAX_PAIRS) return fail(-1, "batch out of range (1..%d)", SSP_MAX_PAIRS);
  const int Hc = h->cfg.height / 8, Wc = h->cfg.width / 8;
  if (Hc * Wc > SAMPLER_MAX_CELLS) return fail(-1, "sampler supports at most %d cells", SAMPLER_MAX_CELLS);
  if (h->cfg.n_match > SAMPLER_MAX_CELLS) return fail(-1, "n_match too large for the device sampler");
  int cap = 2048;
  while (cap < Hc * Wc || cap < h->cfg.n_match) cap <<= 1;
  static AttrOnce attr_once;
  if (attr_once.need()) {
    HIPCHK(hipFuncSetAttribute(reinterpret_cast<const void*>(sample_matches_kernel), hipFuncAttributeMaxDynamicSharedMemorySize,
                               SAMPLER_MAX_CELLS * 12));
  }
  hipLaunchKernelGGL(sample_matches_kernel, dim3(batch), dim3(1024), (size_t)cap * 12, st, homographies_dev, hcell_dev, seed,
                     seed_dev, match_a_dev, match_b_dev, Hc, Wc, h->cfg.n_match, cap);
  const long tot = (long)batch * h->cfg.n_match * h->cfg.n_non;
  hipLaunchKernelGGL(sample_nonmatches_kernel, dim3(cdiv(tot, 256)), dim3(256), 0, st, seed, seed_dev, nonmatch_b_dev, tot, Hc,
                     Wc);
  HIPCHK(hipGetLastError());
  return 0;
}

__global__ void set_seed_kernel(uint64_t* dst, uint64_t v) { *dst = v; }

extern "C" {

int ssp_adam_step_scaled(ssp_handle* h, float lr, int step, float grad_scale, void* stream) {
  if (!h || !h->bound || !h->buf.grads_dev || !h->buf.adam_m_dev || !h->buf.adam_v_dev)
    return fail(-1, "handle not bound with gradient and Adam state buffers");
  if (step < 1) return fail(-1, "Adam step index starts at 1");
  const long n = (long)h->n_params + 3;
  const AdamScalars a = adam_scalars(lr, step);
  hipLaunchKernelGGL(adam_scaled_kernel, dim3(cdiv(n, 256)), dim3(256), 0, (hipStream_t)stream, h->buf.params_dev,
                     h->buf.grads_dev, h->buf.adam_m_dev, h->buf.adam_v_dev, n, a.step_size, a.bc2_sqrt, grad_scale);
  HIPCHK(hipGetLastError());
  return 0;
}

int ssp_handle_set_conv_algo(ssp_handle* h, int algo) {
  if (!h) return fail(-1, "null handle");
  CHK(check_conv_algo(algo));
  h->conv_algo = algo;
  return 0;
}

int ssp_pair_step(ssp_handle* h, const ssp_pair_inputs* in, float* scalars_dev, void* stream) {
  return pair_step_impl(h, in, scalars_dev, 0, (hipStream_t)stream);
}

int ssp_pair_step_phase(ssp_handle* h, const ssp_pair_inputs* in, float* scalars_dev, int phase, void* stream) {
  return pair_step_impl(h, in, scalars_dev, phase, (hipStream_t)stream);
}

size_t ssp_grad_early_offset(const ssp_handle* h) { return h ? h->L[EARLY_SPLIT_LAYER].w_off : 0; }

int ssp_pair_step_graph(ssp_handle* h, const ssp_pair_inputs* in, float* scalars_dev, int phase, int sample_indices,
                        void* stream) {
  if (!h || !h->bound) return fail(-1, "handle not bound");
  if (!in || !scalars_dev) return fail(-1, "null argument");
  hipStream_t st = (hipStream_t)stream;
  if (st == nullptr) return fail(-1, "ssp_pair_step_graph needs a non-default stream (stream capture)");
  if (h->tap_arena != nullptr) return fail(-1, "ssp_pair_step_graph: backward taps are on (ssp_debug_backward_taps); they need the eager step");
  std::vector<unsigned char> key(sizeof(ssp_pair_inputs) + sizeof(void*) + 4 * sizeof(int));
  {
    ssp_pair_inputs k;
    memcpy(&k, in, sizeof(k));
    k.seed = 0;
    memcpy(key.data(), &k, sizeof(k));
    memcpy(key.data() + sizeof(k), &scalars_dev, sizeof(void*));
    const int extra[4] = {phase, sample_indices, h->conv_algo, bf16_fuse_apply_env() ? 1 : 0};
    memcpy(key.data() + sizeof(k) + sizeof(void*), extra, sizeof(extra));
  }
  hipGraphExec_t exec = nullptr;
  for (auto& g : h->graphs)
    if (g.key == key) { exec = g.exec; break; }
  if (exec == nullptr) {
    if (h->prof_family != 0) return fail(-1, "ssp_pair_step_graph: disable ssp_profile_enable before capturing");
    if (h->graphs.size() >= 16) {
      (void)hipGraphExecDestroy(h->graphs.front().exec);
      h->graphs.erase(h->graphs.begin());
    }
    hipGraph_t graph = nullptr;
    HIPCHK(hipStreamBeginCapture(st, hipStreamCaptureModeThreadLocal));
    int rc = 0;
    if (sample_indices && phase != 2) {
      if (!in->match_a_dev || !in->match_b_dev || !in->nonmatch_b_dev) rc = fail(-1, "graph step: index buffers required");
      else rc = sample_indices_impl(h, in->homographies_dev, in->cell_homographies_dev, in->batch, 0, h->graph_seed,
                                    const_cast<int32_t*>(in->match_a_dev),
                                    const_cast<int32_t*>(in->match_b_dev), const_cast<int32_t*>(in->nonmatch_b_dev), st);
    }
    if (rc == 0) rc = pair_step_impl(h, in, scalars_dev, phase, st);
    const hipError_t ce = hipStreamEndCapture(st, &graph);
    if (rc != 0) { if (graph) (void)hipGraphDestroy(graph); return rc; }
    if (ce != hipSuccess) return fail(-2, "hipStreamEndCapture failed: %s", hipGetErrorString(ce));
    const hipError_t ie = hipGraphInstantiate(&exec, graph, nullptr, nullptr, 0);
    (void)hipGraphDestroy(graph);
    if (ie != hipSuccess) return fail(-2, "hipGraphInstantiate failed: %s", hipGetErrorString(ie));
    h->graphs.push_back({key, exec});
  }
  if (sample_indices && phase != 2) {
    hipLaunchKernelGGL(set_seed_kernel, dim3(1), dim3(1), 0, st, h->graph_seed, in->seed);
    HIPCHK(hipGetLastError());
  }
  HIPCHK(hipGraphLaunch(exec, st));
  return 0;
}

int ssp_sample_indices(ssp_handle* h, const float* homographies_dev, int batch, uint64_t seed, int32_t* match_a_dev,
                       int32_t* match_b_dev, int32_t* nonmatch_b_dev, void* stream) {
  return sample_indices_impl(h, homographies_dev, nullptr, batch, seed, nullptr, match_a_dev, match_b_dev, nonmatch_b_dev,
                             (hipStream_t)stream);
}

int ssp_sample_indices_cell(ssp_handle* h, const float* cell_homographies_dev, int batch, uint64_t seed, int32_t* match_a_dev,
                            int32_t* match_b_dev, int32_t* nonmatch_b_dev, void* stream) {
  if (!cell_homographies_dev) return fail(-1, "sample_indices_cell: cell homographies required");
  return sample_indices_impl(h, nullptr, cell_homographies_dev, batch, seed, nullptr, match_a_dev, match_b_dev, nonmatch_b_dev,
                             (hipStream_t)stream);
}

int ssp_op_conv(const float* in_dev, const float* w_oihw_dev, const float* bias_dev, float* out_dev, int n, int hh, int w,
                int cin, int cout, int ksize, int in_mode, const float* in_scale_dev, const float* in_shift_dev,
                double* stats_dev, int transpose_flip, void* workspace_dev, size_t workspace_bytes, void* stream) {
  AlgoScope algo(nullptr);
  if (ksize == 1 && in_mode != 2 && g1_enabled() && g1_fits(cin, cout, (long)n * hh * w, cin, cout, 1)) {
    const size_t img = g1_image_floats(cin, cout) * sizeof(float);
    if (workspace_bytes >= img) {
      hipStream_t st = (hipStream_t)stream;
      float* wpk = reinterpret_cast<float*>(workspace_dev);
      G1PackJobs G;
      G.n = 0;
      int nb = 0;
      g1_add_pack(G, nb, w_oihw_dev, wpk, transpose_flip ? cin : cout, transpose_flip ? cout : cin, transpose_flip ? 1 : 0);
      hipLaunchKernelGGL(pack_g1_kernel, dim3(nb), dim3(256), 0, st, G);
      HIPCHK(hipGetLastError());
      G1Layer y;
      y.in[0] = in_dev; y.in_cs = cin; y.in_co = 0; y.out[0] = out_dev; y.out_cs = cout; y.out_co = 0; y.wpk = wpk; y.bias = bias_dev;
      y.scale[0] = in_scale_dev; y.shift[0] = in_shift_dev; y.stats[0] = stats_dev; y.K = cin; y.N = cout;
      return launch_g1(&y, 1, 1, (long)n * hh * w, in_mode, device_cu_count(), st);
    }
  }
  const bool wino = wino_ok(ksize, cin) && in_mode != 2;
  const int nchunks = cdiv(cin, CK), ncob = cdiv(cout, NB);
  const size_t need = (size_t)ncob * nchunks * pk_taps(ksize) * CK * NB * sizeof(float);
  if (workspace_bytes < need) return fail(-4, "ssp_op_conv workspace too small (%zu < %zu)", workspace_bytes, need);
  if (bf16_path() && ksize == 3 && cin % CK == 0 && in_mode != 2)
    return fail(-3, "ssp_op_conv: conv algorithm 12 has no fp32 3x3 kernel for Cin %% 16 == 0 (use ssp_op_conv_bf16 or another algorithm)");
  hipStream_t st = (hipStream_t)stream;
  float* wpk = reinterpret_cast<float*>(workspace_dev);
  const bool w4 = wino && ksize == 3 && w4_eligible(nullptr, 1, n, hh, w, cin, cout);
  if (!transpose_flip) CHK(launch_pack(w_oihw_dev, wpk, cout, cin, ksize, 0, wino, st, w4));
  else CHK(launch_pack(w_oihw_dev, wpk, cin, cout, ksize, 1, wino, st, w4));
  ConvCall c;
// ... 991 lines not shown
  return n;
}

int ssp_debug_conv_knobs(int ablate, int grid) {
  g_dbg_ablate = ablate; g_dbg_grid = grid;
  return 0;
}

int ssp_debug_backward_taps(ssp_handle* h, float* arena_dev, size_t arena_floats, unsigned layer_mask) {
  if (!h) return fail(-1, "bad argument");
  h->tap_arena = nullptr; h->tap_mask = 0;
  if (arena_dev == nullptr) return 0;
  const unsigned mask = layer_mask & 0xffffu;
  const size_t need = tap_offset(h, mask, 2, 0, 0);
  if (arena_floats < need) return fail(-1, "backward-tap arena holds %zu floats, the layer mask needs %zu", arena_floats, need);
  h->tap_arena = arena_dev; h->tap_mask = mask;
  return 0;
}
size_t ssp_debug_backward_tap_floats(const ssp_handle* h, unsigned layer_mask) {
  return h ? tap_offset(h, layer_mask & 0xffffu, 2, 0, 0) : 0;
}
int ssp_debug_backward_tap(ssp_handle* h, int slot, int layer, int which, size_t* offset, size_t* nfloats, unsigned* route) {
  if (!h || slot < 0 || slot > 1 || layer < 0 || layer >= 16 || which < 0 || which > 1) return fail(-1, "bad argument");
  const size_t n = h->tap_arena != nullptr && (h->tap_mask >> layer & 1) ? tap_floats(h, layer, which) : 0;
  if (offset) *offset = n ? tap_offset(h, h->tap_mask, slot, layer, which) : 0;
  if (nfloats) *nfloats = n;
  if (route) *route = h->tap_route[layer];
  return 0;
}

int ssp_debug_buffer(ssp_handle* h, int slot, const char* name, float** ptr, size_t* nfloats) {
  if (!h || !h->bound || !name || !ptr) return fail(-1, "bad argument");
  Slot& S = h->slot[slot & 1];
  const size_t cells = (size_t)h->cfg.max_batch * (h->cfg.height / 8) * (h->cfg.width / 8);
  std::string n(name);
  float* p = nullptr; size_t cnt = 0;
  if (n == "gP") { p = S.gP; cnt = (size_t)h->cfg.max_batch * h->cfg.height * h->cfg.width * 64; }
  else if (n == "gQ") { p = S.gQ; cnt = (size_t)h->cfg.max_batch * h->cfg.height * h->cfg.width * 64; }
  else if (n == "dsemi") { p = S.dsemi; cnt = cells * 80; }
  else if (n == "ddesc") { p = S.ddesc; cnt = cells * 256; }
  else if (n == "desc") { p = S.desc; cnt = cells * 256; }
  else if (n == "dsout") { p = S.dsout; cnt = cells * h->sout_cs; }
  else if (n[0] == 'Y') { int l = atoi(name + 1); if (l < 0 || l >= h->nlayers) return fail(-1, "bad layer"); p = S.Y[l]; cnt = 0; }
  else if (n[0] == 'A') { int l = atoi(name + 1); if (l < 0 || l >= 8 || !S.Apool[l]) return fail(-1, "no pooled copy of that layer"); p = S.Apool[l]; cnt = 0; }
  else if (n.rfind("scale", 0) == 0) { int l = atoi(name + 5); p = S.bn[l].scale; cnt = h->L[l].cout; }
  else if (n.rfind("shift", 0) == 0) { int l = atoi(name + 5); p = S.bn[l].shift; cnt = h->L[l].cout; }
  else if (n.rfind("mean", 0) == 0) { int l = atoi(name + 4); p = S.bn[l].mean; cnt = h->L[l].cout; }
  else if (n.rfind("invstd", 0) == 0) { int l = atoi(name + 6); p = S.bn[l].invstd; cnt = h->L[l].cout; }
  else return fail(-1, "unknown buffer %s", name);
  *ptr = p;
  if (nfloats) *nfloats = cnt;
  return 0;
}

int ssp_op_dense_loss(const float* desc_a_nhwc_dev, const float* desc_b_nhwc_dev, const float* homographies_dev,
                      const float* valid_dev, int b, int hc, int wc, float lamda_d, float descriptor_dist, int multi_task,
                      float scale, void* scratch_dev, size_t scratch_bytes, float* out3_dev, float* dda_dev,
                      float* ddb_dev, void* stream) {
  const int pc = hc * wc;
  const bool grad = dda_dev != nullptr && ddb_dev != nullptr;
  const size_t need = align_up(sizeof(StepAccum), 256) + (grad ? (size_t)b * pc * pc * sizeof(float) : 0);
  if (scratch_bytes < need) return fail(-4, "ssp_op_dense_loss scratch too small (%zu < %zu)", scratch_bytes, need);
  hipStream_t st = (hipStream_t)stream;
  StepAccum* acc = reinterpret_cast<StepAccum*>(scratch_dev);
  float* coef = grad ? reinterpret_cast<float*>(reinterpret_cast<char*>(scratch_dev) + align_up(sizeof(StepAccum), 256)) : nullptr;
  hipLaunchKernelGGL(dense_op_prep_kernel, dim3(1), dim3(256), 0, st, acc, valid_dev, b * pc, scale);
  DenseArgs da;
  da.da = desc_a_nhwc_dev; da.db = desc_b_nhwc_dev; da.hn = homographies_dev; da.valid = valid_dev; da.coef = coef;
  da.acc = acc; da.B = b; da.Hc = hc; da.Wc = wc; da.lamda_d = lamda_d; da.dist = descriptor_dist; da.multi_task = multi_task;
  hipLaunchKernelGGL(dense_dots_kernel, dim3(cdiv(pc, 64), cdiv(pc, 64), b), dim3(256), 0, st, da);
  if (grad) {
    hipLaunchKernelGGL((dense_grad_kernel<false>), dim3(4, cdiv(pc, 64), b), dim3(256), 0, st, coef, desc_b_nhwc_dev, dda_dev, pc);
    hipLaunchKernelGGL((dense_grad_kernel<true>), dim3(4, cdiv(pc, 64), b), dim3(256), 0, st, coef, desc_a_nhwc_dev, ddb_dev, pc);
  }
  hipLaunchKernelGGL(dense_op_finish_kernel, dim3(1), dim3(1), 0, st, acc, out3_dev, b, pc);
  HIPCHK(hipGetLastError());
  return 0;
}

int ssp_op_sparse_loss(const float* desc_a_nhwc_dev, const float* desc_b_nhwc_dev, const int32_t* match_a_dev,
                       const int32_t* match_b_dev, const int32_t* nonmatch_b_dev, int b, int hc, int wc, int n_match,
                       int n_non, int method, int dist, float coef_pos, float coef_neg, float* dd_a_nhwc_dev, float* dd_b_nhwc_dev,
                       float* out2_dev, void* stream) {
  if (b < 1 || b > SSP_MAX_PAIRS) return fail(-1, "batch out of range (1..%d)", SSP_MAX_PAIRS);
  if ((dd_a_nhwc_dev == nullptr) != (dd_b_nhwc_dev == nullptr)) return fail(-1, "sparse_loss: both gradient pointers or none");
  hipStream_t st = (hipStream_t)stream;
  const bool grad = dd_a_nhwc_dev != nullptr;
  const int dflags = (method != 0 ? DESC_METHOD_1D : 0) | (dist != 0 ? DESC_EUCLIDEAN : 0);
  StepAccum* acc = nullptr;
  float* dots = nullptr;
  HIPCHK(hipMallocAsync((void**)&acc, sizeof(StepAccum), st));
  HIPCHK(hipMemsetAsync(acc, 0, sizeof(StepAccum), st));
  hipLaunchKernelGGL(sparse_op_prep_kernel, dim3(1), dim3(1), 0, st, acc, coef_pos, coef_neg);
  const size_t ncell_floats = (size_t)b * hc * wc * 256;
  const bool euc = (dflags & DESC_EUCLIDEAN) != 0;
  const dim3 dgrid(desc_grid(b, n_match));
  if (grad) {
    HIPCHK(hipMallocAsync((void**)&dots, (size_t)b * n_match * n_non * sizeof(float), st));
    CHK(dev_zero(dd_a_nhwc_dev, ncell_floats * sizeof(float), st));
    CHK(dev_zero(dd_b_nhwc_dev, ncell_floats * sizeof(float), st));
  }
#define SSP_OPD(KERNEL, ...)                                                                  \
  {                                                                                           \
    if (euc) hipLaunchKernelGGL((KERNEL<true>), dgrid, dim3(256), 0, st, __VA_ARGS__);        \
    else hipLaunchKernelGGL((KERNEL<false>), dgrid, dim3(256), 0, st, __VA_ARGS__);           \
  }
  if (grad) {
    if (euc) hipLaunchKernelGGL((desc_match_kernel<true, true>), dgrid, dim3(256), 0, st, desc_a_nhwc_dev, desc_b_nhwc_dev, match_a_dev,
                                match_b_dev, dd_a_nhwc_dev, dd_b_nhwc_dev, acc, b, hc, wc, n_match, dflags);
    else hipLaunchKernelGGL((desc_match_kernel<true, false>), dgrid, dim3(256), 0, st, desc_a_nhwc_dev, desc_b_nhwc_dev, match_a_dev,
                            match_b_dev, dd_a_nhwc_dev, dd_b_nhwc_dev, acc, b, hc, wc, n_match, dflags);
  } else {
    if (euc) hipLaunchKernelGGL((desc_match_kernel<false, true>), dgrid, dim3(256), 0, st, desc_a_nhwc_dev, desc_b_nhwc_dev, match_a_dev,
                                match_b_dev, (float*)nullptr, (float*)nullptr, acc, b, hc, wc, n_match, dflags);
    else hipLaunchKernelGGL((desc_match_kernel<false, false>), dgrid, dim3(256), 0, st, desc_a_nhwc_dev, desc_b_nhwc_dev, match_a_dev,
                            match_b_dev, (float*)nullptr, (float*)nullptr, acc, b, hc, wc, n_match, dflags);
  }
  SSP_OPD(desc_nonmatch_fwd_kernel, desc_a_nhwc_dev, desc_b_nhwc_dev, match_a_dev, nonmatch_b_dev, dots, acc, b, hc, wc, n_match, n_non, dflags)
  if (grad)
    SSP_OPD(desc_nonmatch_bwd_kernel, desc_a_nhwc_dev, desc_b_nhwc_dev, match_a_dev, nonmatch_b_dev, dots, dd_a_nhwc_dev, dd_b_nhwc_dev, acc, b,
            hc, wc, n_match, n_non, dflags)
#undef SSP_OPD
  hipLaunchKernelGGL(sparse_loss_means_kernel, dim3(1), dim3(1), 0, st, acc, out2_dev, b, n_match);
  HIPCHK(hipGetLastError());
  if (dots != nullptr) HIPCHK(hipFreeAsync(dots, st));
  HIPCHK(hipFreeAsync(acc, st));
  return 0;
}

int ssp_op_detector_loss(const float* semi_nhwc_dev, int cs, const float* labels2d_dev, const float* mask2d_dev, int b, int hh,
                         int w, void* scratch_dev, size_t scratch_bytes, float* loss_dev, float* dsemi_nhwc_dev, void* stream) {
  if (hh % 8 || w % 8 || cs < 65) return fail(-1, "detector_loss: H, W multiples of 8 and channel stride >= 65 required");
  const int ncells = b * (hh / 8) * (w / 8);
  const size_t need = align_up(sizeof(StepAccum), 256) + (size_t)(ncells + 65 * 2) * sizeof(float);
  if (scratch_bytes < need) return fail(-4, "ssp_op_detector_loss scratch too small (%zu < %zu)", scratch_bytes, need);
  hipStream_t st = (hipStream_t)stream;
  StepAccum* acc = reinterpret_cast<StepAccum*>(scratch_dev);
  float* cellmask = reinterpret_cast<float*>(reinterpret_cast<char*>(scratch_dev) + align_up(sizeof(StepAccum), 256));
  float* ones = cellmask + ncells;
  hipLaunchKernelGGL(detector_op_prep_kernel, dim3(1), dim3(64), 0, st, acc);
  hipLaunchKernelGGL(fill_affine_identity_kernel, dim3(1), dim3(128), 0, st, ones, 65);
  hipLaunchKernelGGL(cell_mask_kernel, dim3(std::min(cdiv(ncells, 4), 512)), dim3(256), 0, st, mask2d_dev, cellmask,
                     &acc->mask_cnt[0], b, hh, w);
  hipLaunchKernelGGL(detector_loss_kernel, dim3(std::min(cdiv(ncells, 4), 1024)), dim3(256), 0, st, semi_nhwc_dev, ones,
                     ones + 65, labels2d_dev, cellmask, dsemi_nhwc_dev, acc, 0, b, hh, w, cs);
  hipLaunchKernelGGL(detector_op_finish_kernel, dim3(1), dim3(64), 0, st, acc, loss_dev);
  HIPCHK(hipGetLastError());
  return 0;
}

int ssp_op_sem_loss(const float* sout_nhwc_dev, int cs, const int64_t* labels_dev, int b, int hh, int w, int n_classes, int algo,
                    void* scratch_dev, size_t scratch_bytes, float* loss_dev, float* dsout_nhwc_dev, void* stream) {
  if (hh % 8 || w % 8 || cs < n_classes || n_classes < 1) return fail(-1, "sem_loss: H, W multiples of 8 and channel stride >= n_classes required");
  if (algo < 0 || algo > 2) return fail(-1, "sem_loss: algo 0 (the step's choice), 1 or 2");
  if (scratch_bytes < sizeof(StepAccum)) return fail(-4, "ssp_op_sem_loss scratch too small (%zu < %zu)", scratch_bytes, sizeof(StepAccum));
  hipStream_t st = (hipStream_t)stream;
  StepAccum* acc = reinterpret_cast<StepAccum*>(scratch_dev);
  const int hc = hh / 8, wc = w / 8;
  hipLaunchKernelGGL(sem_op_prep_kernel, dim3(1), dim3(64), 0, st, acc);
  hipLaunchKernelGGL(sem_count_kernel, dim3(512, 1), dim3(256), 0, st, labels_dev, labels_dev, (long)b * hh * w, n_classes, acc);
  if (dsout_nhwc_dev != nullptr) CHK(dev_zero(dsout_nhwc_dev, (size_t)b * hc * wc * cs * sizeof(float), st));
  CHK(launch_sem_ce(algo, dsout_nhwc_dev != nullptr, sout_nhwc_dev, labels_dev, dsout_nhwc_dev, acc, 0, b, hc, wc, hh, w, n_classes, cs, st));
  hipLaunchKernelGGL(sem_op_finish_kernel, dim3(1), dim3(64), 0, st, acc, loss_dev);
  HIPCHK(hipGetLastError());
  return 0;
}

int ssp_op_sem_predict(const float* sout_nhwc_dev, int cs, const int64_t* labels_dev, int b, int hh, int w, int n_classes,
                       uint8_t* pred_dev, int64_t* confusion_dev, void* stream) {
  if (!sout_nhwc_dev || b < 1 || hh < 8 || w < 8) return fail(-1, "sem_predict: bad argument");
  if (hh % 8 || w % 8) return fail(-1, "sem_predict: H and W must be multiples of 8 (got %dx%d)", hh, w);
  if (n_classes < 1 || n_classes > SEMP_MAX_C || cs < n_classes)
    return fail(-1, "sem_predict: 1 <= n_classes <= %d and channel stride >= n_classes required (got %d, stride %d)", SEMP_MAX_C, n_classes, cs);
  if (!pred_dev && !confusion_dev) return fail(-1, "sem_predict: neither a class map nor a confusion matrix requested");
  if (confusion_dev && !labels_dev) return fail(-1, "sem_predict: a confusion matrix needs labels");
  const int hc = hh / 8, wc = w / 8;
  const long ntile = (long)b * (hc + 1) * (wc + 1);
  if (ntile > (1L << 30) || (size_t)b * hc * wc * cs > ((size_t)1 << 40)) return fail(-1, "sem_predict: shape too large");
  const int tpw = std::max(SEMP_MIN_TILES, cdiv((int)ntile, SEMP_WAVES));
  const dim3 grid(cdiv(cdiv((int)ntile, tpw), 4)), block(256);
  hipStream_t st = (hipStream_t)stream;
  unsigned long long* conf = reinterpret_cast<unsigned long long*>(confusion_dev);
  if (cs % 4 == 0 && (reinterpret_cast<size_t>(sout_nhwc_dev) & 15) == 0)
    hipLaunchKernelGGL(sem_predict_kernel<true>, grid, block, 0, st, sout_nhwc_dev, labels_dev, pred_dev, conf, b, hc, wc, n_classes, cs, tpw);
  else
    hipLaunchKernelGGL(sem_predict_kernel<false>, grid, block, 0, st, sout_nhwc_dev, labels_dev, pred_dev, conf, b, hc, wc, n_classes, cs, tpw);
  HIPCHK(hipGetLastError());
  return 0;
}

int ssp_sem_predict(ssp_handle* h, int slot, const int64_t* labels_dev, uint8_t* pred_dev, int64_t* confusion_dev, void* stream) {
  if (!h || !h->bound) return fail(-1, "handle not bound");
  if (h->nheads != 3) return fail(-1, "sem_predict: the model has no segmentation head");
  if (slot < 0 || slot > 1) return fail(-1, "sem_predict: slot must be 0 or 1");
  Slot& S = h->slot[slot];
  if (S.N <= 0) return fail(-1, "sem_predict: slot %d holds no forward", slot);
  return ssp_op_sem_predict(S.Y[L_SOUT], h->sout_cs, labels_dev, S.N, S.H, S.W, h->cfg.n_classes, pred_dev, confusion_dev, stream);
}

int ssp_op_labels(const float* labels2d_dev, const float* mask2d_dev, float* target_dev, float* cellmask_dev, int b,
                  int hh, int w, void* stream) {
  if (hh % 8 || w % 8) return fail(-1, "H and W must be multiples of 8");
  hipStream_t st = (hipStream_t)stream;
  const int ncells = b * (hh / 8) * (w / 8);
  if (labels2d_dev && target_dev)
    hipLaunchKernelGGL(labels2dto3d_kernel, dim3(cdiv(ncells, 4)), dim3(256), 0, st, labels2d_dev, target_dev, b, hh, w);
  if (mask2d_dev && cellmask_dev) {
    double* cnt = nullptr;
// ... 11 lines not shown
```

semantic-superpoint_amd/lib.py:

```python
import ctypes as C
import os
from collections import OrderedDict

import numpy as np
import torch

from . import hipbuild as _build

ARCHS = {"SuperPointNet_gauss2": 0, "SuperPointNet_gauss2_ssmall": 1}
SCALAR_NAMES = ["loss", "loss_det", "loss_det_warp", "loss_desc", "loss_sem", "loss_sem_warp", "positive_dist",
                "negative_dist", "eta_det", "eta_desc", "eta_sem"]
N_SCALARS = 16
NREP = 32
SAMPLER_MAX_MATCHES = 8192
PROF = {"none": 0, "conv3x3_fwd": 1, "conv3x3_dgrad": 2, "conv3x3_wgrad": 3, "conv_big_fwd": 4, "conv3x3_all": 5,
        "conv3x3_every": 6}
PROF_KERNELS = ["conv_wino4_kernel", "conv_wino_pipe_kernel", "conv_wino_p2_kernel", "wgrad_wino_kernel", "wgrad_wino4_kernel",
                "other", "conv_bf16_kernel", "wgrad_bf16_kernel"]


class SspConfig(C.Structure):
    _fields_ = [("arch", C.c_int), ("n_classes", C.c_int), ("max_batch", C.c_int), ("height", C.c_int),
                ("width", C.c_int), ("n_match", C.c_int), ("n_non", C.c_int), ("dense_loss", C.c_int)]

# ... 14 lines not shown
                ("dense_lamda_d", C.c_float), ("descriptor_dist", C.c_float), ("cell_homographies_dev", C.c_void_p),
                ("sparse_method", C.c_int), ("sparse_dist", C.c_int)]


class SspHomographyParams(C.Structure):
    _fields_ = [("perspective", C.c_int32), ("scaling", C.c_int32), ("rotation", C.c_int32), ("translation", C.c_int32),
                ("allow_artifacts", C.c_int32), ("n_scales", C.c_int32), ("n_angles", C.c_int32),
                ("scaling_amplitude", C.c_float), ("perspective_amplitude_x", C.c_float),
                ("perspective_amplitude_y", C.c_float), ("patch_ratio", C.c_float), ("max_angle", C.c_float),
                ("translation_overflow", C.c_float)]


class SspPhotometricParams(C.Structure):
    _fields_ = [("struct_size", C.c_uint32), ("random_brightness", C.c_int32), ("random_contrast", C.c_int32),
                ("additive_gaussian_noise", C.c_int32), ("additive_speckle_noise", C.c_int32), ("motion_blur", C.c_int32),
                ("additive_shade", C.c_int32), ("brightness_max_abs_change", C.c_int32),
                ("contrast_lo", C.c_float), ("contrast_hi", C.c_float), ("noise_std_lo", C.c_float), ("noise_std_hi", C.c_float),
                ("impulse_prob_lo", C.c_float), ("impulse_prob_hi", C.c_float), ("shade_nb_ellipses", C.c_int32),
                ("shade_transparency_lo", C.c_float), ("shade_transparency_hi", C.c_float),
                ("shade_kernel_lo", C.c_int32), ("shade_kernel_hi", C.c_int32)]


PHOTO_MAX_ELLIPSES, PHOTO_MAX_KSIZE = 32, 351
(PHOTO_BRIGHTNESS, PHOTO_CONTRAST, PHOTO_SIGMA, PHOTO_IMPULSE_P, PHOTO_BLUR_FLAG, PHOTO_BLUR_W, PHOTO_ELLIPSES, PHOTO_TRANSPARENCY,
 PHOTO_KSIZE, PHOTO_KEY, PHOTO_DRAW_STRIDE) = 0, 1, 2, 3, 4, 5, 14, 174, 175, 176, 180


class SspShapesParams(C.Structure):
    _fields_ = [("struct_size", C.c_uint32), ("gen_h", C.c_int32), ("gen_w", C.c_int32), ("out_h", C.c_int32), ("out_w", C.c_int32),
                ("blur_size", C.c_int32), ("weights", C.c_float * 9),
                ("bg_nb_blobs", C.c_int32), ("bg_min_kernel", C.c_int32), ("bg_max_kernel", C.c_int32),
                ("bg_min_rad_ratio", C.c_float), ("bg_max_rad_ratio", C.c_float),
                ("lines_nb_lines", C.c_int32), ("polygon_max_sides", C.c_int32), ("multi_max_sides", C.c_int32),
                ("multi_nb_polygons", C.c_int32), ("multi_nb_blobs", C.c_int32), ("multi_kernel_lo", C.c_int32),
                ("multi_kernel_hi", C.c_int32), ("ellipses_nb", C.c_int32), ("star_nb_branches", C.c_int32),
                ("checker_max_rows", C.c_int32), ("checker_max_cols", C.c_int32), ("stripes_max_nb_cols", C.c_int32),
                ("checker_transform", C.c_float * 2), ("stripes_transform", C.c_float * 2), ("stripes_min_width_ratio", C.c_float),
                ("cube_min_size_ratio", C.c_float), ("cube_scale", C.c_float * 2), ("cube_trans", C.c_float * 2),
                ("resize_scale_y", C.c_float), ("resize_scale_x", C.c_float), ("gauss_w", C.c_float * 63)]


SHAPES_PRIMITIVES = ["draw_lines", "draw_polygon", "draw_multiple_polygons", "draw_ellipses", "draw_star", "draw_checkerboard",
                     "draw_stripes", "draw_cube", "gaussian_noise"]
SHAPES_MAX_BLOBS, SHAPES_MAX_CMDS, SHAPES_MAX_VERTS, SHAPES_MAX_TEX, SHAPES_MAX_POINTS, SHAPES_MAX_BLUR = 128, 64, 256, 32, 256, 63
(SHAPES_PRIM, SHAPES_THR, SHAPES_KEY, SHAPES_KSIZE, SHAPES_NBLOBS, SHAPES_MEAN0, SHAPES_MEAN, SHAPES_NCMDS, SHAPES_NPOINTS, SHAPES_NVERTS,
 SHAPES_NTEX, SHAPES_BLOBS, SHAPES_CMDS, SHAPES_VERTS, SHAPES_TEX, SHAPES_POINTS, SHAPES_ROW) = (0, 1, 2, 4, 5, 6, 7, 8, 9, 10, 11, 16, 528, 1296,
                                                                                              1808, 2192, 2704)


class SspDetEvalParams(C.Structure):
    _fields_ = [("height", C.c_int32), ("width", C.c_int32), ("remove_zero", C.c_float), ("r2", C.c_int32),
                ("prob_thresh", C.c_float), ("simplified", C.c_int32)]


class SspExportParams(C.Structure):
    _fields_ = [("n_views", C.c_int32), ("height", C.c_int32), ("width", C.c_int32), ("conf_thresh", C.c_float),
                ("nms_dist", C.c_int32), ("border_remove", C.c_int32), ("top_k", C.c_int32), ("subpixel", C.c_int32)]


_lib = None

EXPORTS = ["ssp_last_error", "ssp_create", "ssp_destroy", "ssp_param_count", "ssp_bn_channel_count",
           "ssp_bn_layer_count", "ssp_workspace_bytes", "ssp_bind", "ssp_forward", "ssp_backward", "ssp_zero_grad",
           "ssp_pair_step", "ssp_adam_step", "ssp_sample_indices", "ssp_profile_enable", "ssp_profile_read", "ssp_profile_read_executed",
           "ssp_op_conv", "ssp_op_conv_wgrad", "ssp_op_labels", "ssp_op_sparse_loss", "ssp_op_bn_bwd", "ssp_op_bn_bwd_strided",
           "ssp_debug_buffer", "ssp_debug_conv_knobs", "ssp_set_conv_algo", "ssp_op_warp_image", "ssp_op_erode", "ssp_op_warp_labels",
           "ssp_export_workspace_bytes", "ssp_export_max_points", "ssp_export_points", "ssp_op_homoadapt_views",
           "ssp_op_flatten_detection", "ssp_op_combine_heatmap", "ssp_op_heatmap_points", "ssp_op_soft_argmax_points", "ssp_detector_heatmap", "ssp_op_heatmap_nms", "ssp_op_dense_loss",
           "ssp_op_sample_homographies", "ssp_op_warp_labels_full", "ssp_op_sem_finalize", "ssp_adam_step_scaled",
           "ssp_pair_step_phase", "ssp_grad_early_offset", "ssp_pair_step_graph", "ssp_handle_set_conv_algo",
           "ssp_op_detector_loss", "ssp_debug_occupancy", "ssp_sample_indices_cell", "ssp_op_warp_labels_px",
           "ssp_op_warp_labels_full_px", "ssp_profile_read_kernel", "ssp_op_label_quantize", "ssp_profile_pause", "ssp_op_conv_bf16", "ssp_op_conv_wgrad_bf16", "ssp_op_bn_bwd_bf16", "ssp_build_id",
           "ssp_set_deterministic", "ssp_get_deterministic", "ssp_clock_probe", "ssp_op_sem_loss",
           "ssp_describe_workspace_bytes", "ssp_describe_points", "ssp_op_sample_descriptors", "ssp_match_workspace_bytes",
           "ssp_match_two_way", "ssp_debug_backward_taps", "ssp_debug_backward_tap_floats", "ssp_debug_backward_tap",
           "ssp_eval_repeatability", "ssp_eval_ransac_workspace_bytes", "ssp_eval_ransac",
           "ssp_op_photometric_draw", "ssp_op_photometric_apply",
           "ssp_shapes_workspace_bytes", "ssp_op_shapes_draw", "ssp_op_shapes_render", "ssp_op_warp_points_scatter",
           "ssp_op_sem_predict", "ssp_sem_predict",
           "ssp_track_workspace_bytes", "ssp_op_track_update", "ssp_op_track_select", "ssp_op_track_points",
           "ssp_op_point_classes", "ssp_point_classes", "ssp_filter_workspace_bytes", "ssp_op_filter_points",
           "ssp_match_two_way_classes",
           "ssp_det_eval_workspace_bytes", "ssp_op_det_tp_fp", "ssp_op_det_tp_fp_points", "ssp_det_pr_curve_workspace_bytes",
           "ssp_op_det_pr_curve"]

MATCH_MAX_POINTS = 4096
TRACK_MAX_LENGTH = 16
TRACK_NO_SCORE = 9999.0
CLASS_NONE = 255
DET_EVAL_MAX_R2 = 64
DET_EVAL_STATE_WORDS = 80
DET_EVAL_OUTSIDE = 3
DET_EVAL_HIST = 8
DET_CURVE_TILE = 1024


def load_library(path=None):
    global _lib
    if _lib is not None and path is None:
        return _lib
    path = path or os.environ.get("SSP_HIP_LIB")
    if path is None:
        path = _build.build_locked()
    if not os.path.exists(path):
        raise RuntimeError("libssp_hip.so not found at %s" % path)
    if os.environ.get("SSP_SKIP_ISA_VERIFY") != "1" and not _build.verified(path):
        try:
            _build.verify_and_stamp(path)
        except _build.MissingTool as e:
            raise RuntimeError("%s - cannot check the accumulation-register contract of %s; set SSP_SKIP_ISA_VERIFY=1 to load it "
                               "unchecked" % (e, path)) from e
        except OSError:
            _build.verify_binary(path)
    lib = C.CDLL(path)
    vp, i, f = C.c_void_p, C.c_int, C.c_float
    lib.ssp_last_error.restype = C.c_char_p
    try:
        lib.ssp_build_id.restype = C.c_char_p
        lib.ssp_set_deterministic.argtypes = [C.c_int]
        lib.ssp_get_deterministic.restype = C.c_int
    except AttributeError:
        if os.environ.get("SSP_HIP_LIB") is None:
            raise
    lib.ssp_create.argtypes = [C.POINTER(SspConfig), C.POINTER(vp)]
    lib.ssp_destroy.argtypes = [vp]
    lib.ssp_destroy.restype = None
    for n in ("ssp_param_count", "ssp_bn_channel_count", "ssp_workspace_bytes"):
        getattr(lib, n).argtypes = [vp]
        getattr(lib, n).restype = C.c_size_t
    lib.ssp_bn_layer_count.argtypes = [vp]
    lib.ssp_bind.argtypes = [vp, C.POINTER(SspBuffers), vp]
    lib.ssp_forward.argtypes = [vp, i, vp, i, i, i, i, vp, vp, vp, vp]
    lib.ssp_backward.argtypes = [vp, i, vp, vp, vp, vp]
    lib.ssp_zero_grad.argtypes = [vp, vp]
    lib.ssp_pair_step.argtypes = [vp, C.POINTER(SspPairInputs), vp, vp]
    lib.ssp_adam_step.argtypes = [vp, f, i, vp]
    lib.ssp_adam_step_scaled.argtypes = [vp, f, i, f, vp]
    lib.ssp_pair_step_phase.argtypes = [vp, C.POINTER(SspPairInputs), vp, i, vp]
    lib.ssp_pair_step_graph.argtypes = [vp, C.POINTER(SspPairInputs), vp, i, i, vp]
    lib.ssp_grad_early_offset.argtypes = [vp]
    lib.ssp_grad_early_offset.restype = C.c_size_t
    lib.ssp_handle_set_conv_algo.argtypes = [vp, i]
    lib.ssp_op_detector_loss.argtypes = [vp, i, vp, vp, i, i, i, vp, C.c_size_t, vp, vp, vp]
    try:
        lib.ssp_op_sem_loss.argtypes = [vp, i, vp, i, i, i, i, i, vp, C.c_size_t, vp, vp, vp]
    except AttributeError:
        if os.environ.get("SSP_HIP_LIB") is None:
            raise
    lib.ssp_sample_indices.argtypes = [vp, vp, i, C.c_uint64, vp, vp, vp, vp]
    lib.ssp_sample_indices_cell.argtypes = [vp, vp, i, C.c_uint64, vp, vp, vp, vp]
    lib.ssp_op_warp_labels_px.argtypes = [vp, vp, vp, i, i, i, vp]
    lib.ssp_op_warp_labels_full_px.argtypes = [vp, vp, vp, vp, vp, i, i, i, vp]
    lib.ssp_profile_enable.argtypes = [vp, i]
    lib.ssp_profile_read.argtypes = [vp, C.POINTER(C.c_double), C.POINTER(C.c_int64), C.POINTER(C.c_double),
                                     C.POINTER(C.c_double)]
    lib.ssp_profile_read_executed.argtypes = [vp, C.POINTER(C.c_double)]
    try:
        lib.ssp_profile_pause.argtypes = [vp, i]
    except AttributeError:
        if os.environ.get("SSP_HIP_LIB") is None:
            raise
    try:
        lib.ssp_profile_read_kernel.argtypes = [vp, i, C.POINTER(C.c_double), C.POINTER(C.c_int64), C.POINTER(C.c_double),
                                                C.POINTER(C.c_double), C.POINTER(C.c_double)]
    except AttributeError:
        if os.environ.get("SSP_HIP_LIB") is None:
            raise
    lib.ssp_op_conv.argtypes = [vp, vp, vp, vp, i, i, i, i, i, i, i, vp, vp, vp, i, vp, C.c_size_t, vp]
    lib.ssp_op_conv_wgrad.argtypes = [vp, vp, vp, i, i, i, i, i, i, i, vp, vp, vp, C.c_size_t, vp]
    try:
        lib.ssp_op_conv_bf16.argtypes = [vp, vp, vp, vp, i, i, i, i, i, i, i, vp, vp, vp, i, i, i, vp, vp, vp, C.c_size_t, vp]
        lib.ssp_op_conv_wgrad_bf16.argtypes = [vp, vp, vp, i, i, i, i, i, i, i, vp, vp, i, vp, C.c_size_t, vp]
        lib.ssp_op_bn_bwd_bf16.argtypes = [vp, vp, vp, vp, vp, vp, vp, vp, vp, i, i, i, i, i, i, i, vp]
    except AttributeError:
        if os.environ.get("SSP_HIP_LIB") is None:
            raise
    lib.ssp_debug_buffer.argtypes = [vp, i, C.c_char_p, C.POINTER(vp), C.POINTER(C.c_size_t)]
    if hasattr(lib, "ssp_debug_backward_taps"):
        lib.ssp_debug_backward_taps.argtypes = [vp, vp, C.c_size_t, C.c_uint]
        lib.ssp_debug_backward_tap_floats.argtypes = [vp, C.c_uint]
        lib.ssp_debug_backward_tap_floats.restype = C.c_size_t
        lib.ssp_debug_backward_tap.argtypes = [vp, i, i, i, C.POINTER(C.c_size_t), C.POINTER(C.c_size_t), C.POINTER(C.c_uint)]
    lib.ssp_debug_conv_knobs.argtypes = [i, i]
    lib.ssp_debug_occupancy.argtypes = [i]
    lib.ssp_set_conv_algo.argtypes = [i]
    lib.ssp_op_warp_image.argtypes = [vp, vp, vp, i, i, i, i, vp]
    lib.ssp_op_erode.argtypes = [vp, vp, i, i, i, i, vp]
    lib.ssp_op_warp_labels.argtypes = [vp, vp, vp, i, i, i, vp]
    lib.ssp_op_bn_bwd.argtypes = [vp, vp, vp, vp, vp, vp, vp, vp, vp, i, i, i, i, i, i, vp]
    lib.ssp_op_bn_bwd_strided.argtypes = [vp, vp, vp, vp, vp, vp, vp, vp, vp, i, i, i, i, i, i, i, vp]
    lib.ssp_op_labels.argtypes = [vp, vp, vp, vp, i, i, i, vp]
    lib.ssp_op_sparse_loss.argtypes = [vp, vp, vp, vp, vp, i, i, i, i, i, i, i, C.c_float, C.c_float, vp, vp, vp, vp]
    ep = C.POINTER(SspExportParams)
    lib.ssp_export_workspace_bytes.argtypes = [ep]
    lib.ssp_export_workspace_bytes.restype = C.c_size_t
    lib.ssp_export_max_points.argtypes = [ep]
    lib.ssp_export_points.argtypes = [vp, ep, i] + [C.POINTER(vp)] * 7 + [vp]
    lib.ssp_op_homoadapt_views.argtypes = [vp, vp, vp, vp, i, i, i, vp]
    lib.ssp_op_flatten_detection.argtypes = [vp, vp, vp, i, i, i, vp]
    lib.ssp_op_combine_heatmap.argtypes = [vp, vp, vp, vp, i, i, i, vp]
    lib.ssp_op_heatmap_points.argtypes = [vp, ep, vp, vp, vp, vp]
    lib.ssp_op_soft_argmax_points.argtypes = [vp, vp, vp, i, i, i, vp]
    lib.ssp_detector_heatmap.argtypes = [vp, i, vp, vp]
    lib.ssp_op_heatmap_nms.argtypes = [vp, ep, i, vp, vp, vp, vp, vp]
    lib.ssp_op_sample_homographies.argtypes = [C.c_uint64, C.POINTER(SspHomographyParams), i, vp, vp, vp]
    lib.ssp_op_warp_labels_full.argtypes = [vp, vp, vp, vp, vp, i, i, i, vp]
    lib.ssp_op_sem_finalize.argtypes = [vp, vp, vp, C.c_size_t, i, vp]
    try:
        lib.ssp_op_photometric_draw.argtypes = [C.c_uint64, C.POINTER(SspPhotometricParams), i, i, i, vp, vp]
        lib.ssp_op_photometric_apply.argtypes = [vp, vp, vp, i, i, i, vp]
    except AttributeError:
        if os.environ.get("SSP_HIP_LIB") is None:
            raise
    try:
        sp = C.POINTER(SspShapesParams)
        lib.ssp_shapes_workspace_bytes.argtypes = [sp, i]
        lib.ssp_shapes_workspace_bytes.restype = C.c_size_t
        lib.ssp_op_shapes_draw.argtypes = [C.c_uint64, sp, i, vp, vp]
        lib.ssp_op_shapes_render.argtypes = [vp, sp, i, vp, vp, vp, vp, vp]
        lib.ssp_op_warp_points_scatter.argtypes = [vp, vp, vp, vp, i, i, i, i, vp]
    except AttributeError:
        if os.environ.get("SSP_HIP_LIB") is None:
            raise
    try:
        lib.ssp_op_label_quantize.argtypes = [vp, vp, C.c_size_t, vp]
    except AttributeError:
        if os.environ.get("SSP_HIP_LIB") is None:
            raise
    lib.ssp_op_dense_loss.argtypes = [vp, vp, vp, vp, i, i, i, f, f, i, f, vp, C.c_size_t, vp, vp, vp, vp]
    try:
        lib.ssp_op_sem_predict.argtypes = [vp, i, vp, i, i, i, i, vp, vp, vp]
        lib.ssp_sem_predict.argtypes = [vp, i, vp, vp, vp, vp]
    except AttributeError:
        if os.environ.get("SSP_HIP_LIB") is None:
            raise
    try:
        lib.ssp_describe_workspace_bytes.argtypes = [ep, i]
        lib.ssp_describe_workspace_bytes.restype = C.c_size_t
        lib.ssp_describe_points.argtypes = [vp, i, ep, i, vp, vp, vp, vp, vp]
        lib.ssp_op_sample_descriptors.argtypes = [vp, i, i, i, vp, vp, i, vp, vp]
        lib.ssp_match_workspace_bytes.argtypes = [i, i]
        lib.ssp_match_workspace_bytes.restype = C.c_size_t
        lib.ssp_match_two_way.argtypes = [vp, vp, vp, vp, i, i, i, f, vp, vp, vp, vp]
        lib.ssp_eval_repeatability.argtypes = [vp, vp, vp, vp, i, i, i, vp, vp, i, i, i, C.c_double, vp, vp]
        lib.ssp_eval_ransac_workspace_bytes.argtypes = [i, i]
        lib.ssp_eval_ransac_workspace_bytes.restype = C.c_size_t
        lib.ssp_eval_ransac.argtypes = [vp, vp, i, i, i, vp, vp, vp, vp, vp, vp, vp, vp, vp, vp]
    except AttributeError:
        if os.environ.get("SSP_HIP_LIB") is None:
            raise
    try:
        lib.ssp_track_workspace_bytes.argtypes = [i, i, i]
        lib.ssp_track_workspace_bytes.restype = C.c_size_t
        lib.ssp_op_track_update.argtypes = [vp, vp, vp, vp, vp, vp, vp, vp, i, i, i, vp, vp, vp, vp, vp, vp]
        lib.ssp_op_track_select.argtypes = [vp, vp, vp, vp, i, i, i, vp, vp, vp, vp]
        lib.ssp_op_track_points.argtypes = [vp, vp, vp, vp, i, i, i, i, vp, vp]
    except AttributeError:
        if os.environ.get("SSP_HIP_LIB") is None:
            raise
    try:
        lib.ssp_op_point_classes.argtypes = [vp, i, i, i, i, i, vp, i, vp, i, vp, vp]
        lib.ssp_point_classes.argtypes = [vp, i, i, vp, i, vp, i, vp, vp]
        lib.ssp_filter_workspace_bytes.argtypes = [i, i]
        lib.ssp_filter_workspace_bytes.restype = C.c_size_t
        lib.ssp_op_filter_points.argtypes = [vp, vp, vp, vp, C.POINTER(C.c_uint32), i, i, vp, vp, vp, vp, vp, vp]
        lib.ssp_match_two_way_classes.argtypes = [vp, vp, vp, vp, vp, vp, i, i, i, f, vp, vp, vp, vp]
    except AttributeError:
        if os.environ.get("SSP_HIP_LIB") is None:
            raise
    try:
        dp = C.POINTER(SspDetEvalParams)
        lib.ssp_det_eval_workspace_bytes.argtypes = [dp, i, i]
        lib.ssp_det_eval_workspace_bytes.restype = C.c_size_t
        lib.ssp_op_det_tp_fp.argtypes = [vp, vp, i, dp, i, vp, vp, C.c_int64, vp, vp]
        lib.ssp_op_det_tp_fp_points.argtypes = [vp, vp, i, vp, i, dp, i, vp, vp, C.c_int64, vp, vp]
# ... 697 lines not shown
    return cls


def class_mask(keep=None, drop=None, n_classes=133):
    if (keep is None) == (drop is None):
        raise ValueError("class_mask: exactly one of keep and drop must be given")
    n_classes = int(n_classes)
    if not 1 <= n_classes <= CLASS_NONE:
        raise ValueError("class_mask: 1 <= n_classes <= %d required (got %d)" % (CLASS_NONE, n_classes))
    ids = [int(c) for c in (keep if keep is not None else drop)]
    for c in ids:
        if not 0 <= c < n_classes:
            raise ValueError("class_mask: class id %d outside [0, %d)" % (c, n_classes))
    kept = set(ids) if keep is not None else set(range(n_classes)) - set(ids)
    words = [0] * 8
    for c in kept:
        words[c >> 5] |= 1 << (c & 31)
    return tuple(words)


def op_filter_points(pts, count, desc, cls, mask):
    lib = load_library()
    for t, nm in ((pts, "pts"), (count, "count"), (desc, "desc"), (cls, "cls")):
        _need_gpu(t, nm)
    mask = [int(w) for w in mask]
    if len(mask) != 8 or any(not 0 <= w < 1 << 32 for w in mask):
        raise ValueError("mask must be eight 32-bit words (class_mask)")
    if pts.dtype != torch.float32 or pts.dim() != 3 or pts.shape[2] != 5:
        raise ValueError("pts must be float32 [n, cap, 5], got %s %s" % (pts.dtype, tuple(pts.shape)))
    n, cap = pts.shape[0], pts.shape[1]
    if desc.dtype != torch.float32 or tuple(desc.shape) != (n, cap, 256):
        raise ValueError("desc must be float32 [%d, %d, 256]" % (n, cap))
    if cls.dtype != torch.uint8 or tuple(cls.shape) != (n, cap) or count.dtype != torch.int32 or count.numel() != n:
        raise ValueError("cls must be uint8 [%d, %d] and count int32 [%d]" % (n, cap, n))
    dev = pts.device
    out = {"pts": torch.empty_like(pts), "count": torch.zeros(n, dtype=torch.int32, device=dev),
           "desc": torch.empty_like(desc), "cls": torch.empty_like(cls)}
    if n == 0 or cap == 0:
        return out
    wsb = lib.ssp_filter_workspace_bytes(n, cap)
    if wsb == 0:
        _check(-1)
    ws = torch.empty(wsb, dtype=torch.uint8, device=dev)
    with torch.cuda.device(dev):
        _check(lib.ssp_op_filter_points(_ptr(pts), _ptr(count), _ptr(desc), _ptr(cls), (C.c_uint32 * 8)(*mask), n, cap,
                                        _ptr(out["pts"]), _ptr(out["count"]), _ptr(out["desc"]), _ptr(out["cls"]), _ptr(ws),
                                        _stream()))
    return out


def sem_metrics(confusion):
    m = confusion.detach().cpu().numpy() if torch.is_tensor(confusion) else np.asarray(confusion)
    if m.ndim != 2 or m.shape[0] != m.shape[1]:
        raise ValueError("confusion must be a square matrix, got shape %s" % (tuple(m.shape),))
    m = m.astype(np.float64)
    tp, row, col = np.diag(m), m.sum(1), m.sum(0)
    n_pixels = m.sum()
    union = row + col - tp
    present = union > 0
    iou = np.full(m.shape[0], np.nan)
    iou[present] = tp[present] / union[present]
    return {"n_pixels": int(n_pixels), "pixel_acc": float(tp.sum() / n_pixels) if n_pixels > 0 else float("nan"),
            "iou": iou, "miou": float(iou[present].mean()) if present.any() else float("nan"),
            "classes_present": int(present.sum())}


def op_detector_loss(semi_nchw, labels2d, mask2d, grad=True):
    lib = load_library()
    _need_gpu(semi_nchw, "semi")
    B, c, Hc, Wc = semi_nchw.shape
    assert c == 65
    dev = semi_nchw.device
    x = torch.zeros(B, Hc, Wc, 80, dtype=torch.float32, device=dev)
    x[..., :65] = semi_nchw.permute(0, 2, 3, 1)
    d = torch.empty_like(x) if grad else None
    out = torch.zeros(1, dtype=torch.float32, device=dev)
    scratch = torch.empty(65536 + 4 * (B * Hc * Wc + 256), dtype=torch.uint8, device=dev)
    with torch.cuda.device(dev):
        _check(lib.ssp_op_detector_loss(_ptr(x), 80, _ptr(labels2d.contiguous()), _ptr(mask2d.contiguous()), B, Hc * 8, Wc * 8,
                                        _ptr(scratch), scratch.numel(), _ptr(out), _ptr(d), _stream()))
    return float(out.item()), (d[..., :65].permute(0, 3, 1, 2).contiguous() if grad else None)


def op_sparse_loss(desc_a_nchw, desc_b_nchw, match_a, match_b, nonmatch_b, method="2d", dist="cos", grad=None):
    lib = load_library()
    _need_gpu(desc_a_nchw, "desc")
    B, D, Hc, Wc = desc_a_nchw.shape
    a = desc_a_nchw.permute(0, 2, 3, 1).contiguous()
    b = desc_b_nchw.permute(0, 2, 3, 1).contiguous()
    out = torch.zeros(2, dtype=torch.float32, device=a.device)
    da = torch.full_like(a, float("nan")) if grad is not None else None
    db = torch.full_like(b, float("nan")) if grad is not None else None
    cp, cn = grad if grad is not None else (0.0, 0.0)
    with torch.cuda.device(a.device):
        _check(lib.ssp_op_sparse_loss(_ptr(a), _ptr(b), _ptr(match_a), _ptr(match_b), _ptr(nonmatch_b), B, Hc, Wc,
                                      match_a.shape[1], nonmatch_b.shape[1] // match_a.shape[1], int(method != "2d"), int(dist != "cos"),
                                      float(cp), float(cn), _ptr(da), _ptr(db), _ptr(out), _stream()))
    torch.cuda.synchronize()
    if grad is None:
        return float(out[0]), float(out[1])
    return float(out[0]), float(out[1]), da.permute(0, 3, 1, 2).contiguous(), db.permute(0, 3, 1, 2).contiguous()


def op_dense_loss(desc_a_nchw, desc_b_nchw, homographies, mask_valid, lamda_d=250.0, descriptor_dist=4.0, grad=None):
    lib = load_library()
    _need_gpu(desc_a_nchw, "desc")
    B, D, Hc, Wc = desc_a_nchw.shape
    dev = desc_a_nchw.device
    a = desc_a_nchw.permute(0, 2, 3, 1).contiguous()
    b = desc_b_nchw.permute(0, 2, 3, 1).contiguous()
    hm = homographies.to(dev, torch.float32).contiguous()
    mv = mask_valid.to(dev, torch.float32).reshape(B, Hc * Wc).contiguous()
    out = torch.zeros(3, dtype=torch.float32, device=dev)
    da = torch.empty_like(a) if grad else None
    db = torch.empty_like(b) if grad else None
    scratch = torch.empty(65536 + (B * (Hc * Wc) ** 2 * 4 if grad else 0), dtype=torch.uint8, device=dev)
    with torch.cuda.device(dev):
        _check(lib.ssp_op_dense_loss(_ptr(a), _ptr(b), _ptr(hm), _ptr(mv), B, Hc, Wc, float(lamda_d), float(descriptor_dist),
                                     int(bool(grad and grad[0] == "multi_task")), float(grad[1]) if grad else 0.0,
                                     _ptr(scratch), scratch.numel(), _ptr(out), _ptr(da), _ptr(db), _stream()))
    o = out.cpu().tolist()
    if not grad:
        return o[0], o[1], o[2]
    return (o[0], o[1], o[2]), da.permute(0, 3, 1, 2).contiguous(), db.permute(0, 3, 1, 2).contiguous()


def op_bn_bwd(y_nhwc, dout_nhwc, gamma, scale, shift, mean, invstd, relu=True, pool=False):
    lib = load_library()
    _need_gpu(y_nhwc, "y")
    N, H, W, cs = y_nhwc.shape
    Cc = gamma.numel()
    dev = y_nhwc.device
    stats4 = torch.cat([scale, shift, mean, invstd]).contiguous()
    dy = torch.zeros_like(y_nhwc) if cs != Cc else torch.empty_like(y_nhwc)
    dg, db, dbias = (torch.zeros(Cc, dtype=torch.float32, device=dev) for _ in range(3))
    sums = torch.zeros(NREP * 2 * Cc, dtype=torch.float64, device=dev)
    with torch.cuda.device(dev):
        _check(lib.ssp_op_bn_bwd_strided(_ptr(y_nhwc), _ptr(dout_nhwc), _ptr(gamma), _ptr(stats4), _ptr(dy), _ptr(dg),
                                         _ptr(db), _ptr(dbias), _ptr(sums), N, H, W, Cc, cs, int(relu), int(pool), _stream()))
    return dy, dg, db, dbias


def op_bn_bwd_bf16(y_nhwc, dout_nhwc, gamma, scale, shift, mean, invstd, pool=False):
    lib = load_library()
    _need_gpu(y_nhwc, "y")
    if y_nhwc.dtype != torch.bfloat16 or dout_nhwc.dtype != torch.bfloat16:
        raise RuntimeError("y and dout must be bfloat16")
    N, H, W, cs = y_nhwc.shape
    Cc = gamma.numel()
    dev = y_nhwc.device
    stats4 = torch.cat([scale, shift, mean, invstd]).contiguous()
    dy = torch.zeros_like(y_nhwc)
    dg, db, dbias = (torch.zeros(Cc, dtype=torch.float32, device=dev) for _ in range(3))
    sums = torch.zeros(NREP * 2 * Cc, dtype=torch.float64, device=dev)
    with torch.cuda.device(dev):
        _check(lib.ssp_op_bn_bwd_bf16(_ptr(y_nhwc), _ptr(dout_nhwc), _ptr(gamma), _ptr(stats4), _ptr(dy), _ptr(dg), _ptr(db),
                                      _ptr(dbias), _ptr(sums), N, H, W, Cc, cs, 1, int(pool), _stream()))
    return dy, dg, db, dbias


def op_warp_image(img, inv_h, nearest=False):
    lib = load_library()
    _need_gpu(img, "img")
    inv_h = inv_h.to(img.device, torch.float32).contiguous()
    B, _, H, W = img.shape
    out = torch.empty_like(img)
    with torch.cuda.device(img.device):
        _check(lib.ssp_op_warp_image(_ptr(img), _ptr(inv_h), _ptr(out), B, H, W, int(bool(nearest)), _stream()))
    return out


def op_erode(mask, radius):
    lib = load_library()
    _need_gpu(mask, "mask")
    B, _, H, W = mask.shape
    out = torch.empty_like(mask)
    with torch.cuda.device(mask.device):
        _check(lib.ssp_op_erode(_ptr(mask), _ptr(out), B, H, W, int(radius), _stream()))
    return out


def op_warp_labels(labels, hn, exact=True):
    lib = load_library()
    _need_gpu(labels, "labels")
# ... 665 lines not shown
```

Before: 2518.

## Replace atomic scatter of match gradients with CSR gather in descriptor backward

Measured after the change: 2553, median of 6. 1.01x the previous value.

```diff
diff --git a/include/ssp_hip.h b/include/ssp_hip.h
--- a/include/ssp_hip.h
+++ b/include/ssp_hip.h
@@ -337,6 +337,11 @@
                        const int32_t* match_b_dev, const int32_t* nonmatch_b_dev, int b, int hc, int wc, int n_match,
                        int n_non, int method, int dist, float coef_pos, float coef_neg, float* dd_a_nhwc_dev, float* dd_b_nhwc_dev,
                        float* out2_dev, void* stream);
+int ssp_op_sparse_loss_path(const float* desc_a_nhwc_dev, const float* desc_b_nhwc_dev, const int32_t* match_a_dev,
+                            const int32_t* match_b_dev, const int32_t* nonmatch_b_dev, int b, int hc, int wc, int n_match,
+                            int n_non, int method, int dist, float coef_pos, float coef_neg, float* dd_a_nhwc_dev, float* dd_b_nhwc_dev,
+                            float* out2_dev, int gather, int32_t* csr_off_dev, int32_t* csr_match_dev, float* csr_weight_dev,
+                            void* stream);
 
 int ssp_op_dense_loss(const float* desc_a_nhwc_dev, const float* desc_b_nhwc_dev, const float* homographies_dev,
                       const float* valid_dev, int b, int hc, int wc, float lamda_d, float descriptor_dist, int multi_task,
diff --git a/semantic-superpoint_amd/csrc/bn_kernels.hip.h b/semantic-superpoint_amd/csrc/bn_kernels.hip.h
--- a/semantic-superpoint_amd/csrc/bn_kernels.hip.h
+++ b/semantic-superpoint_amd/csrc/bn_kernels.hip.h
@@ -790,12 +790,59 @@
   if (lane == 0) inv_norm[wave] = inv;
 }
 
+struct DescGather {
+  const int32_t* off;
+  const int32_t* match;
+  const float* weight;
+  const float* rows;
+  int cells, n_match;
+};
+__device__ __forceinline__ float4 desc_gather_cell(const DescGather& G, int cell, int side, int lane, float4 g) {
+  const int img = cell / G.cells, c = cell - img * G.cells;
+  const int list = img * 2 + side;
+  const int32_t* off = G.off + (size_t)list * (G.cells + 1);
+  const int e0 = off[c], e1 = off[c + 1];
+  const int32_t* em = G.match + (size_t)list * 4 * G.n_match;
+  const float* ew = G.weight + (size_t)list * 4 * G.n_match;
+  const float* rows = G.rows + ((size_t)img * G.n_match * 2 + side) * 256 + lane * 4;
+  for (int b0 = e0; b0 < e1; b0 += 64) {
+    const int n = min(64, e1 - b0);
+    const int le = b0 + min(lane, n - 1);
+    const int ml = em[le];
+    const int wl = lane < n ? __float_as_int(ew[le]) : 0;
+    for (int i = 0; i < n; i += 4) {
+      float4 r[4];
+      float w[4];
+#pragma unroll
+      for (int u = 0; u < 4; ++u) {
+        const int s = min(i + u, 63);
+        w[u] = __int_as_float(__builtin_amdgcn_readlane(wl, s));
+        r[u] = *reinterpret_cast<const float4*>(rows + (size_t)__builtin_amdgcn_readlane(ml, s) * 512);
+      }
+#pragma unroll
+      for (int u = 0; u < 4; ++u) {
+        g.x = fmaf(w[u], r[u].x, g.x); g.y = fmaf(w[u], r[u].y, g.y); g.z = fmaf(w[u], r[u].z, g.z); g.w = fmaf(w[u], r[u].w, g.w);
+      }
+    }
+  }
+  return g;
+}
+__global__ __launch_bounds__(256) void desc_gather_kernel(float* __restrict__ d0, float* __restrict__ d1, int ncells, DescGather G) {
+  float* __restrict__ d = blockIdx.y != 0 ? d1 : d0;
+  const int wave = (blockIdx.x * blockDim.x + threadIdx.x) >> 6;
+  const int lane = threadIdx.x & 63;
+  if (wave >= ncells) return;
+  float4* p = reinterpret_cast<float4*>(d + (size_t)wave * 256 + lane * 4);
+  *p = desc_gather_cell(G, wave, (int)blockIdx.y, lane, *p);
+}
+
 __global__ __launch_bounds__(256) void desc_normalize_bwd_kernel(const float* __restrict__ desc0,
                                                                  const float* __restrict__ inv_norm0,
                                                                  float* __restrict__ d0, int ncells,
                                                                  const float* __restrict__ desc1 = nullptr,
                                                                  const float* __restrict__ inv_norm1 = nullptr,
-                                                                 float* __restrict__ d1 = nullptr) {
+                                                                 float* __restrict__ d1 = nullptr,
+                                                                 DescGather G = DescGather{nullptr, nullptr, nullptr, nullptr, 0, 0}) {
   const bool v1 = blockIdx.y != 0;
   const float* __restrict__ desc = v1 ? desc1 : desc0;
   const float* __restrict__ inv_norm = v1 ? inv_norm1 : inv_norm0;
@@ -805,6 +852,7 @@
   if (wave >= ncells) return;
   const float4 n = *reinterpret_cast<const float4*>(desc + (size_t)wave * 256 + lane * 4);
   float4 g = *reinterpret_cast<const float4*>(d + (size_t)wave * 256 + lane * 4);
+  if (G.off != nullptr) g = desc_gather_cell(G, wave, v1 ? 1 : 0, lane, g);
   float s = n.x * g.x + n.y * g.y + n.z * g.z + n.w * g.w;
 #pragma unroll
   for (int o = 32; o > 0; o >>= 1) s += __shfl_xor(s, o);
diff --git a/semantic-superpoint_amd/csrc/loss_kernels.hip.h b/semantic-superpoint_amd/csrc/loss_kernels.hip.h
--- a/semantic-superpoint_amd/csrc/loss_kernels.hip.h
+++ b/semantic-superpoint_amd/csrc/loss_kernels.hip.h
@@ -220,13 +220,14 @@
   const int k = (slot - round * bpi) * 4 + (threadIdx.x >> 6);
   return (img < B && k < n_match) ? img * n_match + k : -1;
 }
-template <bool BWD, bool EUC = false>
+template <bool BWD, bool EUC = false, bool GATHER = false>
 __global__ __launch_bounds__(256) void desc_match_kernel(const float* __restrict__ desc_a, const float* __restrict__ desc_b,
                                                          const int32_t* __restrict__ match_a,
                                                          const int32_t* __restrict__ match_b, float* __restrict__ dd_a,
                                                          float* __restrict__ dd_b, StepAccum* __restrict__ acc, int B,
-                                                         int Hc, int Wc, int n_match, int flags) {
-  const DetTarget t_a = det_resolve(dd_a), t_b = det_resolve(dd_b);
+                                                         int Hc, int Wc, int n_match, int flags, float* __restrict__ g_rows = nullptr) {
+  const DetTarget t_a = GATHER ? DetTarget{nullptr, nullptr} : det_resolve(dd_a);
+  const DetTarget t_b = GATHER ? DetTarget{nullptr, nullptr} : det_resolve(dd_b);
   int img;
   const int w = desc_wave_of_block(B, n_match, img);
   const int lane = threadIdx.x & 63;
@@ -264,7 +265,16 @@
     term = wave_sum(q);
   }
   if (lane == 0) acc_add_loss(&acc->pos_sum[img * 16 + ((w >> 2) & 15)], (double)term);
-  if (BWD && (euc || term > 0.f)) {
+  if (BWD && GATHER) {
+    const bool on = euc || term > 0.f;
+    const float c = on ? acc->coef_pos / ((float)n_match * (float)B) * (euc ? 2.f : -1.f) : 0.f;
+    float* ga = g_rows + (size_t)w * 512 + lane;
+#pragma unroll
+    for (int j = 0; j < 4; ++j) {
+      ga[64 * j] = on ? c * (euc ? va[j] - vb[j] : vb[j]) : 0.f;
+      ga[256 + 64 * j] = on ? c * (euc ? vb[j] - va[j] : va[j]) : 0.f;
+    }
+  } else if (BWD && (euc || term > 0.f)) {
     const float c = acc->coef_pos / ((float)n_match * (float)B) * (euc ? 2.f : -1.f);
 #pragma unroll
     for (int k = 0; k < 4; ++k) {
@@ -277,6 +287,86 @@
         for (int j = 0; j < 4; ++j) facc_add(t_b, dd_b + base + (size_t)ib[k] * 256 + 64 * j, wb[k] * c * (euc ? vb[j] - va[j] : va[j]));
       }
     }
+  }
+}
+
+static inline size_t desc_csr_lds_bytes(int cells, int n_match) { return ((size_t)2 * cells + 1 + (size_t)8 * n_match) * 4; }
+constexpr int DESC_CSR_THREADS = 1024;
+__device__ __forceinline__ int csr_cell(int c, int cells) { return min(max(c, 0), cells - 1); }
+__global__ __launch_bounds__(DESC_CSR_THREADS) void desc_csr_kernel(const int32_t* __restrict__ match_a, const int32_t* __restrict__ match_b,
+                                                                    int32_t* __restrict__ off_out, int32_t* __restrict__ match_out,
+                                                                    float* __restrict__ weight_out, int Hc, int Wc, int n_match,
+                                                                    int flags) {
+  extern __shared__ __align__(16) int csr_lds[];
+  __shared__ int part[DESC_CSR_THREADS];
+  const int cells = Hc * Wc;
+  int* off = csr_lds;
+  int* cur = off + cells + 1;
+  int* tm = cur + cells;
+  float* tw = reinterpret_cast<float*>(tm + 4 * n_match);
+  const int img = blockIdx.x, side = blockIdx.y, list = img * 2 + side;
+  const int32_t* __restrict__ mt = (side ? match_b : match_a) + (size_t)img * n_match;
+  const bool m1d = (flags & DESC_METHOD_1D) != 0;
+  const int tid = threadIdx.x, nt = blockDim.x;
+  for (int c = tid; c <= cells; c += nt) off[c] = 0;
+  __syncthreads();
+  for (int k = tid; k < n_match; k += nt) {
+    const Bilin b = m1d ? bilin_cell(mt[k]) : bilin_setup(mt[k], Hc, Wc);
+    const int ci[4] = {csr_cell(b.i00, cells), csr_cell(b.i01, cells), csr_cell(b.i10, cells), csr_cell(b.i11, cells)};
+    const float cw[4] = {b.w00, b.w01, b.w10, b.w11};
+#pragma unroll
+    for (int q = 0; q < 4; ++q)
+      if (cw[q] != 0.f) atomicAdd(&off[ci[q] + 1], 1);
+  }
+  __syncthreads();
+  const int per = (cells + nt - 1) / nt;
+  const int c0 = min(tid * per, cells), c1 = min(c0 + per, cells);
+  int sum = 0;
+  for (int c = c0; c < c1; ++c) sum += off[c + 1];
+  part[tid] = sum;
+  __syncthreads();
+  for (int o = 1; o < nt; o <<= 1) {
+    const int v = tid >= o ? part[tid - o] : 0;
+    __syncthreads();
+    part[tid] += v;
+    __syncthreads();
+  }
+  int run = part[tid] - sum;
+  for (int c = c0; c < c1; ++c) {
+    cur[c] = run;
+    run += off[c + 1];
+    off[c + 1] = run;
+  }
+  __syncthreads();
+  int32_t* __restrict__ go = off_out + (size_t)list * (cells + 1);
+  for (int c = tid; c <= cells; c += nt) go[c] = off[c];
+  for (int k = tid; k < n_match; k += nt) {
+    const Bilin b = m1d ? bilin_cell(mt[k]) : bilin_setup(mt[k], Hc, Wc);
+    const int ci[4] = {csr_cell(b.i00, cells), csr_cell(b.i01, cells), csr_cell(b.i10, cells), csr_cell(b.i11, cells)};
+    const float cw[4] = {b.w00, b.w01, b.w10, b.w11};
+#pragma unroll
+    for (int q = 0; q < 4; ++q)
+      if (cw[q] != 0.f) {
+        const int p = atomicAdd(&cur[ci[q]], 1);
+        tm[p] = k;
+        tw[p] = cw[q];
+      }
+  }
+  __syncthreads();
+  int32_t* __restrict__ gm = match_out + (size_t)list * 4 * n_match;
+  float* __restrict__ gw = weight_out + (size_t)list * 4 * n_match;
+  const int total = off[cells];
+  for (int p = tid; p < total; p += nt) {
+    int lo = 0, hi = cells - 1;
+    while (lo < hi) {
+      const int mid = (lo + hi + 1) >> 1;
+      if (off[mid] <= p) lo = mid; else hi = mid - 1;
+    }
+    const int b0 = off[lo], b1 = off[lo + 1], mk = tm[p];
+    int rank = 0;
+    for (int q = b0; q < b1; ++q) rank += tm[q] < mk ? 1 : 0;
+    gm[b0 + rank] = mk;
+    gw[b0 + rank] = tw[p];
   }
 }
 
diff --git a/semantic-superpoint_amd/csrc/ssp.hip b/semantic-superpoint_amd/csrc/ssp.hip
--- a/semantic-superpoint_amd/csrc/ssp.hip
+++ b/semantic-superpoint_amd/csrc/ssp.hip
@@ -168,6 +168,10 @@
   bool bf16_fuse_apply = true;
   StepAccum* accum;
   float* dots;
+  bool desc_gather = true;
+  int32_t *csr_off = nullptr, *csr_match = nullptr;
+  float* csr_weight = nullptr;
+  float* g_rows = nullptr;
   float* dense_coef;
   int sout_cs;
   int conv_algo;
@@ -362,6 +366,12 @@
   h->accum = c.take<StepAccum>(1);
   h->graph_seed = c.take<uint64_t>(1);
   h->dots = c.take<float>((size_t)B * h->cfg.n_match * h->cfg.n_non);
+  if (h->desc_gather) {
+    h->csr_off = c.take<int32_t>((size_t)B * 2 * ((size_t)(H / 8) * (W / 8) + 1));
+    h->csr_match = c.take<int32_t>((size_t)B * 2 * 4 * h->cfg.n_match);
+    h->csr_weight = c.take<float>((size_t)B * 2 * 4 * h->cfg.n_match);
+    h->g_rows = c.take_skewed<float>((size_t)B * h->cfg.n_match * 2 * 256);
+  }
   {
     const size_t pc = (size_t)(H / 8) * (W / 8);
     h->dense_coef = h->cfg.dense_loss ? c.take_skewed<float>((size_t)std::min(B, 64) * pc * pc) : nullptr;
@@ -1121,6 +1131,7 @@
 static int flush_wgrad_reduce_bf16(ssp_handle* h, hipStream_t st) { return h->rq_bf16 != nullptr ? h->rq_bf16->flush(st) : 0; }
 
 static int ensure_aux_stream(ssp_handle* h);
+static bool desc_gather_env();
 
 struct DetHostRegion { float* lo; size_t n; long long* shadow; const ssp_handle* owner; };
 static std::vector<DetHostRegion> g_det_regions;
@@ -1259,6 +1270,7 @@
   if (h->cfg.n_match <= 0) h->cfg.n_match = 1000;
   if (h->cfg.n_non <= 0) h->cfg.n_non = 100;
   h->conv_algo = g_default_conv_algo;
+  h->desc_gather = desc_gather_env();
   h->rq_bf16 = new WredBQueue();
   AlgoScope algo(h);
   build_layers(h);
@@ -2555,6 +2567,10 @@
 
 }
 
+static bool desc_gather_env() {
+  static const int v = getenv("SSP_DESC_GATHER") ? atoi(getenv("SSP_DESC_GATHER")) : 1;
+  return v != 0;
+}
 static int sem_xc_env() {
   static const int v = [] { const char* e = getenv("SSP_SEM_XC"); return e ? atoi(e) : 1; }();
   return v;
@@ -2589,6 +2605,19 @@
   return 0;
 }
 
+static int launch_desc_csr(const int32_t* match_a, const int32_t* match_b, int32_t* off, int32_t* em, float* ew, int B, int Hc, int Wc,
+                           int n_match, int dflags, hipStream_t st) {
+  const size_t lds = desc_csr_lds_bytes(Hc * Wc, n_match);
+  constexpr size_t lds_max = 128 * 1024;
+  if (lds > lds_max) return fail(-1, "desc_csr: %d cells x %d matches need %zu B of LDS (> %zu)", Hc * Wc, n_match, lds, lds_max);
+  static AttrOnce attr_once;
+  if (attr_once.need())
+    HIPCHK(hipFuncSetAttribute(reinterpret_cast<const void*>(desc_csr_kernel), hipFuncAttributeMaxDynamicSharedMemorySize, (int)lds_max));
+  hipLaunchKernelGGL(desc_csr_kernel, dim3(B, 2), dim3(DESC_CSR_THREADS), lds, st, match_a, match_b, off, em, ew, Hc, Wc, n_match, dflags);
+  HIPCHK(hipGetLastError());
+  return 0;
+}
+
 static int pair_step_impl(ssp_handle* h, const ssp_pair_inputs* in, float* scalars_dev, int phase, hipStream_t st_in) {
   void* stream = st_in;
   if (!h || !h->bound) return fail(-1, "handle not bound");
@@ -2628,7 +2657,11 @@
   const float* masks[2] = {in->valid_mask_dev, in->warped_valid_mask_dev};
   const int64_t* sems[2] = {in->semantic_dev, in->warped_semantic_dev};
   const bool zero_dsout = semantic && in->train;
+  const bool gather = h->desc_gather && in->train && use_desc && !dense;
+  const int dflags = (in->sparse_method != 0 ? DESC_METHOD_1D : 0) | (in->sparse_dist != 0 ? DESC_EUCLIDEAN : 0);
   auto label_kernels = [&](hipStream_t se) -> int {
+    if (gather)
+      CHK(launch_desc_csr(in->match_a_dev, in->match_b_dev, h->csr_off, h->csr_match, h->csr_weight, B, Hc, Wc, h->cfg.n_match, dflags, se));
     hipLaunchKernelGGL(cell_mask_kernel, dim3(std::min(cdiv(ncells, 4), 512), nv), dim3(256), 0, se, masks[0], h->slot[0].cellmask,
                        &h->accum->mask_cnt[0], B, H, W, masks[nv - 1], h->slot[nv - 1].cellmask, &h->accum->mask_cnt[nv - 1]);
     if (semantic)
@@ -2683,7 +2716,6 @@
     HIPCHK(hipGetLastError());
   } else if (use_desc) {
     Slot &A = h->slot[0], &Bs = h->slot[1];
-    const int dflags = (in->sparse_method != 0 ? DESC_METHOD_1D : 0) | (in->sparse_dist != 0 ? DESC_EUCLIDEAN : 0);
     const bool euc = (dflags & DESC_EUCLIDEAN) != 0;
     const dim3 dgrid(desc_grid(B, h->cfg.n_match));
 #define SSP_DESC(KERNEL, ...)                                                                 \
@@ -2706,15 +2738,22 @@
         CHK(dev_zero(A.ddesc, (size_t)ncells * 256 * sizeof(float), sd));
         CHK(dev_zero(Bs.ddesc, (size_t)ncells * 256 * sizeof(float), sd));
       }
-      SSP_DESC_MATCH(true, A.desc, Bs.desc, in->match_a_dev, in->match_b_dev, A.ddesc, Bs.ddesc, h->accum, B, Hc, Wc, h->cfg.n_match, dflags)
+      if (gather) {
+        if (euc) hipLaunchKernelGGL((desc_match_kernel<true, true, true>), dgrid, dim3(256), 0, sd, A.desc, Bs.desc, in->match_a_dev, in->match_b_dev,
+                                    (float*)nullptr, (float*)nullptr, h->accum, B, Hc, Wc, h->cfg.n_match, dflags, h->g_rows);
+        else hipLaunchKernelGGL((desc_match_kernel<true, false, true>), dgrid, dim3(256), 0, sd, A.desc, Bs.desc, in->match_a_dev, in->match_b_dev,
+                                (float*)nullptr, (float*)nullptr, h->accum, B, Hc, Wc, h->cfg.n_match, dflags, h->g_rows);
+      } else
+        SSP_DESC_MATCH(true, A.desc, Bs.desc, in->match_a_dev, in->match_b_dev, A.ddesc, Bs.ddesc, h->accum, B, Hc, Wc, h->cfg.n_match, dflags)
       SSP_DESC(desc_nonmatch_bwd_kernel, A.desc, Bs.desc, in->match_a_dev, in->nonmatch_b_dev, h->dots, A.ddesc, Bs.ddesc, h->accum, B, Hc, Wc,
                h->cfg.n_match, h->cfg.n_non, dflags)
 #undef SSP_DESC
 #undef SSP_DESC_MATCH
       CHK(det_fold(A.ddesc, sd));
       CHK(det_fold(Bs.ddesc, sd));
+      const DescGather dg = {gather ? h->csr_off : nullptr, h->csr_match, h->csr_weight, h->g_rows, Hc * Wc, h->cfg.n_match};
       hipLaunchKernelGGL(desc_normalize_bwd_kernel, dim3(cdiv(ncells, 4), 2), dim3(256), 0, sd, A.desc, A.inv_norm, A.ddesc, ncells,
-                         Bs.desc, Bs.inv_norm, Bs.ddesc);
+                         Bs.desc, Bs.inv_norm, Bs.ddesc, dg);
     }
     HIPCHK(hipGetLastError());
   }
@@ -2813,14 +2852,15 @@
   hipStream_t st = (hipStream_t)stream;
   if (st == nullptr) return fail(-1, "ssp_pair_step_graph needs a non-default stream (stream capture)");
   if (h->tap_arena != nullptr) return fail(-1, "ssp_pair_step_graph: backward taps are on (ssp_debug_backward_taps); they need the eager step");
-  std::vector<unsigned char> key(sizeof(ssp_pair_inputs) + sizeof(void*) + 4 * sizeof(int));
+  std::vector<unsigned char> key(sizeof(ssp_pair_inputs) + sizeof(void*) + 5 * sizeof(int));
   {
     ssp_pair_inputs k;
     memcpy(&k, in, sizeof(k));
     k.seed = 0;
     memcpy(key.data(), &k, sizeof(k));
     memcpy(key.data() + sizeof(k), &scalars_dev, sizeof(void*));
-    const int extra[4] = {phase, sample_indices, h->conv_algo, bf16_fuse_apply_env() ? 1 : 0};
+    const int extra[5] = {phase, sample_indices, h->conv_algo, bf16_fuse_apply_env() ? 1 : 0,
+                          h->desc_gather ? 1 : 0};
     memcpy(key.data() + sizeof(k) + sizeof(void*), extra, sizeof(extra));
   }
   hipGraphExec_t exec = nullptr;
@@ -3978,6 +4018,15 @@
                        const int32_t* match_b_dev, const int32_t* nonmatch_b_dev, int b, int hc, int wc, int n_match,
                        int n_non, int method, int dist, float coef_pos, float coef_neg, float* dd_a_nhwc_dev, float* dd_b_nhwc_dev,
                        float* out2_dev, void* stream) {
+  return ssp_op_sparse_loss_path(desc_a_nhwc_dev, desc_b_nhwc_dev, match_a_dev, match_b_dev, nonmatch_b_dev, b, hc, wc, n_match, n_non, method,
+                                 dist, coef_pos, coef_neg, dd_a_nhwc_dev, dd_b_nhwc_dev, out2_dev, -1, nullptr, nullptr, nullptr, stream);
+}
+
+int ssp_op_sparse_loss_path(const float* desc_a_nhwc_dev, const float* desc_b_nhwc_dev, const int32_t* match_a_dev,
+                            const int32_t* match_b_dev, const int32_t* nonmatch_b_dev, int b, int hc, int wc, int n_match,
+                            int n_non, int method, int dist, float coef_pos, float coef_neg, float* dd_a_nhwc_dev, float* dd_b_nhwc_dev,
+                            float* out2_dev, int gather, int32_t* csr_off_dev, int32_t* csr_match_dev, float* csr_weight_dev,
+                            void* stream) {
   if (b < 1 || b > SSP_MAX_PAIRS) return fail(-1, "batch out of range (1..%d)", SSP_MAX_PAIRS);
   if ((dd_a_nhwc_dev == nullptr) != (dd_b_nhwc_dev == nullptr)) return fail(-1, "sparse_loss: both gradient pointers or none");
   hipStream_t st = (hipStream_t)stream;
@@ -3991,17 +4040,36 @@
   const size_t ncell_floats = (size_t)b * hc * wc * 256;
   const bool euc = (dflags & DESC_EUCLIDEAN) != 0;
   const dim3 dgrid(desc_grid(b, n_match));
+  const bool use_gather = grad && (gather < 0 ? desc_gather_env() : gather != 0);
+  const bool own_csr = csr_off_dev == nullptr || csr_match_dev == nullptr || csr_weight_dev == nullptr;
+  if (!own_csr && !use_gather) return fail(-1, "sparse_loss: the corner lists exist on the gather path with gradients only");
+  int32_t *csr_off = csr_off_dev, *csr_match = csr_match_dev;
+  float *csr_weight = csr_weight_dev, *g_rows = nullptr;
   if (grad) {
     HIPCHK(hipMallocAsync((void**)&dots, (size_t)b * n_match * n_non * sizeof(float), st));
     CHK(dev_zero(dd_a_nhwc_dev, ncell_floats * sizeof(float), st));
     CHK(dev_zero(dd_b_nhwc_dev, ncell_floats * sizeof(float), st));
   }
+  if (use_gather) {
+    if (own_csr) {
+      HIPCHK(hipMallocAsync((void**)&csr_off, (size_t)b * 2 * ((size_t)hc * wc + 1) * sizeof(int32_t), st));
+      HIPCHK(hipMallocAsync((void**)&csr_match, (size_t)b * 2 * 4 * n_match * sizeof(int32_t), st));
+      HIPCHK(hipMallocAsync((void**)&csr_weight, (size_t)b * 2 * 4 * n_match * sizeof(float), st));
+    }
+    HIPCHK(hipMallocAsync((void**)&g_rows, (size_t)b * n_match * 2 * 256 * sizeof(float), st));
+    CHK(launch_desc_csr(match_a_dev, match_b_dev, csr_off, csr_match, csr_weight, b, hc, wc, n_match, dflags, st));
+  }
 #define SSP_OPD(KERNEL, ...)                                                                  \
   {                                                                                           \
     if (euc) hipLaunchKernelGGL((KERNEL<true>), dgrid, dim3(256), 0, st, __VA_ARGS__);        \
     else hipLaunchKernelGGL((KERNEL<false>), dgrid, dim3(256), 0, st, __VA_ARGS__);           \
   }
-  if (grad) {
+  if (use_gather) {
+    if (euc) hipLaunchKernelGGL((desc_match_kernel<true, true, true>), dgrid, dim3(256), 0, st, desc_a_nhwc_dev, desc_b_nhwc_dev, match_a_dev,
+                                match_b_dev, (float*)nullptr, (float*)nullptr, acc, b, hc, wc, n_match, dflags, g_rows);
+    else hipLaunchKernelGGL((desc_match_kernel<true, false, true>), dgrid, dim3(256), 0, st, desc_a_nhwc_dev, desc_b_nhwc_dev, match_a_dev,
+                            match_b_dev, (float*)nullptr, (float*)nullptr, acc, b, hc, wc, n_match, dflags, g_rows);
+  } else if (grad) {
     if (euc) hipLaunchKernelGGL((desc_match_kernel<true, true>), dgrid, dim3(256), 0, st, desc_a_nhwc_dev, desc_b_nhwc_dev, match_a_dev,
                                 match_b_dev, dd_a_nhwc_dev, dd_b_nhwc_dev, acc, b, hc, wc, n_match, dflags);
     else hipLaunchKernelGGL((desc_match_kernel<true, false>), dgrid, dim3(256), 0, st, desc_a_nhwc_dev, desc_b_nhwc_dev, match_a_dev,
@@ -4017,9 +4085,19 @@
     SSP_OPD(desc_nonmatch_bwd_kernel, desc_a_nhwc_dev, desc_b_nhwc_dev, match_a_dev, nonmatch_b_dev, dots, dd_a_nhwc_dev, dd_b_nhwc_dev, acc, b,
             hc, wc, n_match, n_non, dflags)
 #undef SSP_OPD
+  if (use_gather) {
+    const DescGather dg = {csr_off, csr_match, csr_weight, g_rows, hc * wc, n_match};
+    hipLaunchKernelGGL(desc_gather_kernel, dim3(cdiv((long)b * hc * wc, 4), 2), dim3(256), 0, st, dd_a_nhwc_dev, dd_b_nhwc_dev, b * hc * wc, dg);
+  }
   hipLaunchKernelGGL(sparse_loss_means_kernel, dim3(1), dim3(1), 0, st, acc, out2_dev, b, n_match);
   HIPCHK(hipGetLastError());
   if (dots != nullptr) HIPCHK(hipFreeAsync(dots, st));
+  if (g_rows != nullptr) HIPCHK(hipFreeAsync(g_rows, st));
+  if (use_gather && own_csr) {
+    HIPCHK(hipFreeAsync(csr_off, st));
+    HIPCHK(hipFreeAsync(csr_match, st));
+    HIPCHK(hipFreeAsync(csr_weight, st));
+  }
   HIPCHK(hipFreeAsync(acc, st));
   return 0;
 }
diff --git a/semantic-superpoint_amd/lib.py b/semantic-superpoint_amd/lib.py
--- a/semantic-superpoint_amd/lib.py
+++ b/semantic-superpoint_amd/lib.py
@@ -120,7 +120,7 @@
            "ssp_op_point_classes", "ssp_point_classes", "ssp_filter_workspace_bytes", "ssp_op_filter_points",
            "ssp_match_two_way_classes",
            "ssp_det_eval_workspace_bytes", "ssp_op_det_tp_fp", "ssp_op_det_tp_fp_points", "ssp_det_pr_curve_workspace_bytes",
-           "ssp_op_det_pr_curve"]
+           "ssp_op_det_pr_curve", "ssp_op_sparse_loss_path"]
 
 MATCH_MAX_POINTS = 4096
 TRACK_MAX_LENGTH = 16
@@ -229,6 +229,11 @@
     lib.ssp_op_bn_bwd_strided.argtypes = [vp, vp, vp, vp, vp, vp, vp, vp, vp, i, i, i, i, i, i, i, vp]
     lib.ssp_op_labels.argtypes = [vp, vp, vp, vp, i, i, i, vp]
     lib.ssp_op_sparse_loss.argtypes = [vp, vp, vp, vp, vp, i, i, i, i, i, i, i, C.c_float, C.c_float, vp, vp, vp, vp]
+    try:
+        lib.ssp_op_sparse_loss_path.argtypes = [vp, vp, vp, vp, vp, i, i, i, i, i, i, i, C.c_float, C.c_float, vp, vp, vp, i, vp, vp, vp, vp]
+    except AttributeError:
+        if os.environ.get("SSP_HIP_LIB") is None:
+            raise
     ep = C.POINTER(SspExportParams)
     lib.ssp_export_workspace_bytes.argtypes = [ep]
     lib.ssp_export_workspace_bytes.restype = C.c_size_t
@@ -1092,7 +1097,7 @@
     return float(out.item()), (d[..., :65].permute(0, 3, 1, 2).contiguous() if grad else None)
 
 
-def op_sparse_loss(desc_a_nchw, desc_b_nchw, match_a, match_b, nonmatch_b, method="2d", dist="cos", grad=None):
+def op_sparse_loss(desc_a_nchw, desc_b_nchw, match_a, match_b, nonmatch_b, method="2d", dist="cos", grad=None, gather=None, csr=False):
     lib = load_library()
     _need_gpu(desc_a_nchw, "desc")
     B, D, Hc, Wc = desc_a_nchw.shape
@@ -1102,14 +1107,28 @@
     da = torch.full_like(a, float("nan")) if grad is not None else None
     db = torch.full_like(b, float("nan")) if grad is not None else None
     cp, cn = grad if grad is not None else (0.0, 0.0)
+    n_match = match_a.shape[1]
+    lists = None
+    if csr:
+        lists = (torch.zeros(B, 2, Hc * Wc + 1, dtype=torch.int32, device=a.device),
+                 torch.full((B, 2, 4 * n_match), -1, dtype=torch.int32, device=a.device),
+                 torch.full((B, 2, 4 * n_match), float("nan"), dtype=torch.float32, device=a.device))
     with torch.cuda.device(a.device):
-        _check(lib.ssp_op_sparse_loss(_ptr(a), _ptr(b), _ptr(match_a), _ptr(match_b), _ptr(nonmatch_b), B, Hc, Wc,
-                                      match_a.shape[1], nonmatch_b.shape[1] // match_a.shape[1], int(method != "2d"), int(dist != "cos"),
-                                      float(cp), float(cn), _ptr(da), _ptr(db), _ptr(out), _stream()))
+        if gather is None and not csr:
+            _check(lib.ssp_op_sparse_loss(_ptr(a), _ptr(b), _ptr(match_a), _ptr(match_b), _ptr(nonmatch_b), B, Hc, Wc,
+                                          n_match, nonmatch_b.shape[1] // n_match, int(method != "2d"), int(dist != "cos"),
+                                          float(cp), float(cn), _ptr(da), _ptr(db), _ptr(out), _stream()))
+        else:
+            _check(lib.ssp_op_sparse_loss_path(_ptr(a), _ptr(b), _ptr(match_a), _ptr(match_b), _ptr(nonmatch_b), B, Hc, Wc,
+                                               n_match, nonmatch_b.shape[1] // n_match, int(method != "2d"), int(dist != "cos"),
+                                               float(cp), float(cn), _ptr(da), _ptr(db), _ptr(out),
+                                               -1 if gather is None else int(bool(gather)), _ptr(lists[0]) if csr else None,
+                                               _ptr(lists[1]) if csr else None, _ptr(lists[2]) if csr else None, _stream()))
     torch.cuda.synchronize()
     if grad is None:
         return float(out[0]), float(out[1])
-    return float(out[0]), float(out[1]), da.permute(0, 3, 1, 2).contiguous(), db.permute(0, 3, 1, 2).contiguous()
+    res = (float(out[0]), float(out[1]), da.permute(0, 3, 1, 2).contiguous(), db.permute(0, 3, 1, 2).contiguous())
+    return res + (lists,) if csr else res
 
 
 def op_dense_loss(desc_a_nchw, desc_b_nchw, homographies, mask_valid, lamda_d=250.0, descriptor_dist=4.0, grad=None):
```
